# humansensinglab/AGenDA

Hardware: AMD Instinct MI355X
Metric: 512x512 images/sec + DAAM heatmaps, 50 DDIM steps, SD-1.5 (higher is better)
Workload: dtype bf16

## Files before the change

### agenda_amd/_lib.py

```python
from __future__ import annotations

import ctypes as C
import os

_HERE = os.path.dirname(os.path.abspath(__file__))
LIB_PATH = os.environ.get("AGD_LIB") or os.path.join(_HERE, "libagenda_hip.so")
AGD_MAX_LEVELS = 8
AGD_N_CLASSES = 11


class AgdConfig(C.Structure):
    _fields_ = [
        ("struct_size", C.c_int),
        ("in_channels", C.c_int), ("out_channels", C.c_int), ("n_levels", C.c_int),
        ("block_out_channels", C.c_int * AGD_MAX_LEVELS),
        ("down_cross", C.c_int * AGD_MAX_LEVELS),
        ("num_heads", C.c_int * AGD_MAX_LEVELS),
        ("layers_per_block", C.c_int), ("cross_attention_dim", C.c_int),
        ("use_linear_projection", C.c_int), ("norm_num_groups", C.c_int),
        ("vae_latent_channels", C.c_int), ("vae_out_channels", C.c_int), ("vae_n_levels", C.c_int),
        ("vae_block_out_channels", C.c_int * AGD_MAX_LEVELS),
        ("vae_layers_per_block", C.c_int), ("vae_norm_num_groups", C.c_int),
        ("vae_scaling_factor", C.c_float),
        ("max_tokens", C.c_int),
# ... 66 lines not shown
    "agd_inpaint_clear": (C.c_int, [_P]),
    "agd_ip2p_prepare_hw": (C.c_int, [_P, _P, C.c_int, C.c_int, C.c_int, C.c_int, _P, _P]),
    "agd_ip2p_set_hw": (C.c_int, [_P, _P, C.c_int, C.c_int, C.c_int, C.c_float, _P]),
    "agd_ip2p_clear": (C.c_int, [_P]),
    "agd_adapter_configure": (C.c_int, [_P, C.POINTER(AgdAdapterConfig)]),
    "agd_adapter_set_cond_hw": (C.c_int, [_P, _P, C.c_int, C.c_int, C.c_int, C.c_int, _P]),
    "agd_adapter_features": (C.c_int, [_P, _P]),
    "agd_adapter_set_schedule": (C.c_int, [_P, C.POINTER(C.c_float), C.c_int]),
    "agd_adapter_clear": (C.c_int, [_P]),
    "agd_adapter_add_counts": (C.c_int, [_P, C.POINTER(C.c_longlong)]),
    "agd_ip_adapter_begin": (C.c_int, [_P, C.c_int, C.c_int]),
    "agd_ip_adapter_tensor": (C.c_int, [_P, C.c_char_p, _P, C.c_int, C.c_int, C.POINTER(C.c_longlong)]),
    "agd_ip_adapter_commit": (C.c_int, [_P]),
    "agd_ip_adapter_unload": (C.c_int, [_P]),
    "agd_ip_adapter_set": (C.c_int, [_P, _P, C.c_int, C.c_float, _P]),
    "agd_ip_adapter_clear": (C.c_int, [_P]),
    "agd_ip_adapter_tokens": (C.c_int, [_P, _P]),
    "agd_ip_adapter_block": (C.c_int, [_P, C.c_char_p, _P, C.c_int, C.c_int, C.c_int, _P, _P]),
    "agd_ip_adapter_counts": (C.c_int, [_P, C.POINTER(C.c_longlong)]),
    "agd_image_encoder_begin": (C.c_int, [_P, C.POINTER(AgdVisionConfig)]),
    "agd_image_encoder_tensor": (C.c_int, [_P, C.c_char_p, _P, C.c_int, C.c_int, C.POINTER(C.c_longlong)]),
    "agd_image_encoder_commit": (C.c_int, [_P]),
    "agd_image_encoder_unload": (C.c_int, [_P]),
    "agd_image_embeds": (C.c_int, [_P, _P, C.c_int, C.c_int, C.c_int, _P, _P]),
    "agd_gligen_configure": (C.c_int, [_P, C.POINTER(AgdGligenConfig)]),
    "agd_gligen_set": (C.c_int, [_P, _P, _P, _P, C.c_int, _P]),
    "agd_gligen_set_schedule": (C.c_int, [_P, C.POINTER(C.c_int), C.c_int]),
    "agd_gligen_clear": (C.c_int, [_P]),
    "agd_gligen_objs": (C.c_int, [_P, _P]),
    "agd_gligen_fuser": (C.c_int, [_P, C.c_char_p, _P, C.c_int, C.c_int, C.c_int, _P, _P]),
    "agd_lora_add": (C.c_int, [_P, C.c_char_p, _P, _P, C.c_int, C.c_float]),
    "agd_lora_set_scale": (C.c_int, [_P, C.c_float, _P]),
    "agd_lora_clear": (C.c_int, [_P]),
    "agd_lora_count": (C.c_int, [_P]),
    "agd_lora_scale": (C.c_float, [_P]),
    "agd_unet_forward": (C.c_int, [_P, _P, C.c_int, C.c_int, C.c_float, _P, _P]),
    "agd_unet_forward_ts": (C.c_int, [_P, _P, C.c_int, C.c_int, C.POINTER(C.c_float), _P, _P]),
    "agd_cfg_ddim_step": (C.c_int, [_P, _P, _P, C.c_int, C.c_int, C.c_float, C.c_float, C.c_float, _P]),
    "agd_denoise": (C.c_int, [_P, _P, C.c_int, C.c_int, C.c_int, C.POINTER(C.c_float), C.POINTER(C.c_float),
                              C.POINTER(C.c_float), C.c_float, _P]),
    "agd_denoise_plms": (C.c_int, [_P, _P, C.c_int, C.c_int, C.c_int, C.POINTER(C.c_float), C.POINTER(C.c_float),
                                   C.POINTER(C.c_float), C.c_float, _P]),
    "agd_denoise_dpm": (C.c_int, [_P, _P, C.c_int, C.c_int, C.c_int, C.POINTER(C.c_float), C.POINTER(C.c_float), C.c_float, _P]),
    "agd_vae_decode": (C.c_int, [_P, _P, C.c_int, C.c_int, _P, _P, _P]),
    "agd_vae_encode": (C.c_int, [_P, _P, C.c_int, C.c_int, _P, _P, _P]),
    "agd_safety_scores_hw": (C.c_int, [_P, _P, C.c_int, C.c_int, C.c_int, _P, _P, _P]),
    "agd_controlnet_set_cond_hw": (C.c_int, [_P, _P, C.c_int, C.c_int, C.c_int, C.c_int, _P]),
    "agd_controlnet_residuals_hw": (C.c_int, [_P, _P, C.c_int, C.c_int, C.c_int, C.c_float, C.c_float, C.c_int, _P, C.POINTER(C.c_longlong), _P]),
    "agd_inpaint_prepare_hw": (C.c_int, [_P, _P, C.c_int, _P, C.c_int, C.c_int, C.c_int, C.c_int, _P, _P, _P, _P]),
    "agd_inpaint_set_hw": (C.c_int, [_P, _P, C.c_int, _P, C.c_int, _P, C.c_int, C.c_int, C.c_int, _P]),
    "agd_unet_forward_hw": (C.c_int, [_P, _P, C.c_int, C.c_int, C.c_int, C.c_float, _P, _P]),
    "agd_unet_forward_ts_hw": (C.c_int, [_P, _P, C.c_int, C.c_int, C.c_int, C.POINTER(C.c_float), _P, _P]),
    "agd_cfg_ddim_step_hw": (C.c_int, [_P, _P, _P, C.c_int, C.c_int, C.c_int, C.c_float, C.c_float, C.c_float, _P]),
    "agd_denoise_hw": (C.c_int, [_P, _P, C.c_int, C.c_int, C.c_int, C.c_int, C.POINTER(C.c_float), C.POINTER(C.c_float),
                                 C.POINTER(C.c_float), C.c_float, _P]),
    "agd_denoise_plms_hw": (C.c_int, [_P, _P, C.c_int, C.c_int, C.c_int, C.c_int, C.POINTER(C.c_float), C.POINTER(C.c_float),
                                      C.POINTER(C.c_float), C.c_float, _P]),
    "agd_denoise_dpm_hw": (C.c_int, [_P, _P, C.c_int, C.c_int, C.c_int, C.c_int, C.POINTER(C.c_float), C.POINTER(C.c_float), C.c_float, _P]),
    "agd_vae_decode_hw": (C.c_int, [_P, _P, C.c_int, C.c_int, C.c_int, _P, _P, _P]),
    "agd_vae_encode_hw": (C.c_int, [_P, _P, C.c_int, C.c_int, C.c_int, _P, _P, _P]),
    "agd_record_reset_hw": (C.c_int, [_P, C.c_int, C.c_int, C.c_int, _P]),
    "agd_set_option": (C.c_int, [_P, C.c_char_p, C.c_int]),
    "agd_record_config": (C.c_int, [_P, C.c_int, C.c_int, C.c_int]),
    "agd_record_reset": (C.c_int, [_P, C.c_int, C.c_int, _P]),
    "agd_daam_global": (C.c_int, [_P, C.c_int, C.c_int, _P, _P]),
    "agd_hook_global": (C.c_int, [_P, _P, _P]),
    "agd_hook_count": (C.c_int, [_P]),
    "agd_hook_last_map": (C.c_int, [_P, _P, C.c_int, _P]),
    "agd_cross_attn": (C.c_int, [_P, C.c_char_p, _P, _P, C.c_int, C.c_int, C.c_int, _P, C.c_int, _P]),
    "agd_attn_processor": (C.c_int, [_P, C.c_char_p, _P, _P, _P, C.c_int, C.c_int, C.c_int, _P, C.c_int, _P]),
    "agd_hook_reset": (C.c_int, [_P, C.c_int, C.c_int, _P]),
    "agd_hook_num_maps": (C.c_int, [_P]),
    "agd_hook_map_dims": (C.c_int, [_P, C.c_int, C.POINTER(C.c_int)]),
    "agd_hook_map": (C.c_int, [_P, C.c_int, _P, _P]),
    "agd_op_attn_reg_loss": (C.c_int, [_P, C.c_int, C.c_int, C.c_int, _P, _P, _P, C.c_float, _P, _P, _P]),
    "agd_attn_processor_backward": (C.c_int, [_P, C.c_char_p, _P, _P, _P, _P, C.c_int, C.c_int, C.c_int, C.c_int, _P, _P, _P]),
    "agd_op_conv2d": (C.c_int, [_P, _P, _P, _P] + [C.c_int] * 9 + [_P]),
    "agd_op_conv2d_ex": (C.c_int, [_P, _P, _P, _P] + [C.c_int] * 10 + [_P]),
    "agd_op_linear": (C.c_int, [_P, _P, _P, _P, _P, C.c_int, C.c_int, C.c_int, C.c_int, _P]),
    "agd_op_groupnorm": (C.c_int, [_P, _P, _P, _P, C.c_int, C.c_int, C.c_int, C.c_int, C.c_float, C.c_int, _P]),
    "agd_op_conv_groupnorm": (C.c_int, [_P] * 6 + [C.c_int] * 6 + [C.c_float, C.c_int, C.c_int, _P]),
    "agd_op_layernorm": (C.c_int, [_P, _P, _P, _P, C.c_int, C.c_int, C.c_float, _P]),
    "agd_op_ff_fused": (C.c_int, [_P] * 8 + [C.c_int, C.c_int, C.c_float, _P]),
    "agd_op_attn_chain": (C.c_int, [_P] * 9 + [C.c_int] * 5 + [C.c_float, _P]),
    "agd_op_xattn_premul": (C.c_int, [_P] * 9 + [C.c_int] * 5 + [C.c_float, _P]),
    "agd_op_attention": (C.c_int, [_P, _P, _P, _P, C.c_int, C.c_int, C.c_int, C.c_int, C.c_int, C.c_float, _P, _P]),
    "agd_op_attention_headsum": (C.c_int, [_P, _P, _P, _P, C.c_int, C.c_int, C.c_int, C.c_int, C.c_int, C.c_float, _P, _P]),
    "agd_op_bicubic_clamp_mean": (C.c_int, [_P, C.c_int, C.c_int, C.c_int, C.c_int, _P, _P]),
    "agd_op_heatmap_u8": (C.c_int, [_P, C.c_int, C.c_int, _P, _P]),
    "agd_op_resize_u8_pil": (C.c_int, [_P, C.c_int, C.c_int, C.c_int, C.c_int, C.c_int, C.c_int, _P, _P]),
    "agd_op_stack_heatmaps": (C.c_int, [_P, _P, _P, C.c_longlong, _P, _P, _P]),
    "agd_op_window_gather": (C.c_int, [_P, _P] + [C.c_int] * 8 + [_P]),
    "agd_op_window_mean": (C.c_int, [_P, _P] + [C.c_int] * 6 + [_P]),
    "agd_denoise_panorama": (C.c_int, [_P, _P] + [C.c_int] * 7 + [C.POINTER(C.c_float)] * 3 + [C.c_float, _P]),
    "agd_daam_global_panorama": (C.c_int, [_P, C.c_int, C.c_int, _P, _P]),
    "agd_freeu_set": (C.c_int, [_P] + [C.c_float] * 4),
    "agd_freeu_clear": (C.c_int, [_P]),
    "agd_freeu_counts": (C.c_int, [_P, C.POINTER(C.c_longlong)]),
    "agd_op_freeu": (C.c_int, [_P, _P, _P, _P] + [C.c_int] * 5 + [C.c_float, C.c_float, _P]),
    "agd_profile_begin": (C.c_int, [_P]),
    "agd_profile_end": (C.c_int, [_P, C.POINTER(C.c_double), C.POINTER(C.c_double), C.POINTER(C.c_longlong)]),
    "agd_profile_end_ex": (C.c_int, [_P, C.c_double, C.c_double] + [C.POINTER(C.c_double)] * 5 + [C.POINTER(C.c_longlong)]),
    "agd_profile_class_name": (C.c_char_p, [C.c_int]),
    "agd_version": (C.c_char_p, []),
}

EXPORTS = tuple(_SIGS.keys())
_lib = None


def load():
    global _lib
    if _lib is not None:
        return _lib
    if not os.path.exists(LIB_PATH):
        raise AgendaHipError(
            f"{LIB_PATH} not found: build it with `python -c 'import __graft_entry__ as g; g.build()'` "
            "or `make -C agenda_amd/csrc`. There is no CPU fallback.")
    lib = C.CDLL(LIB_PATH)
    for name, (res, args) in _SIGS.items():
        fn = getattr(lib, name)
        fn.restype = res
        fn.argtypes = args
    _lib = lib
    return lib


def check(rc: int, ctx=None, what: str = ""):
    if rc != 0:
        msg = load().agd_last_error(ctx)
        raise AgendaHipError(f"{what} failed (rc={rc}): {msg.decode() if msg else '?'}")


def ptr(t):
    if t is None:
        return None
    assert t.is_contiguous(), "tensor must be contiguous"
    return C.c_void_p(t.data_ptr())


def current_stream_ptr():
    import torch
    return C.c_void_p(torch.cuda.current_stream().cuda_stream)
```

### agenda_amd/csrc/kernels.h

```cpp
#pragma once
#include "common.h"

#define AGD_MAX_DEVICES 16
struct SplitKWs { float* p = nullptr; size_t cap = 0; };

struct IgemmP {
  const bf16_t* sc0 = nullptr; const bf16_t* sc1 = nullptr; int sc_C0 = 0, sc_C1 = 0;
  int ups4 = 0;
  const bf16_t* src0; const bf16_t* src1;
  int C0, C1;
  int Hin, Win, Hout, Wout;
  int ksize, stride, pad, up;
  const bf16_t* W;
  const float* bias; int bias_mode;
  const float* rowadd; int rowadd_ld;
  const bf16_t* residual; int ldr;
  void* out; int out_f32; int ldo;
  int M, N, K;
  float alpha;
  int geglu;
  int act;
  int batch;
  long long sA0, sA1, sW, sO, sR;
  const bf16_t* zero_page;
  SplitKWs* ws;
  float* splitk_ws;
  int colstat_rows;
  float* colstat_out;
  float* rowstat_out; int rowstat_slots;
  const float* ln_stats; int ln_slots; const float* ln_cs; float ln_invC, ln_eps;
  int* cfg_out;
  int w_per_image;
  int wmajor;
  int warm;
  int halo;
  int p8;
  const float* gn_gamma; const float* gn_beta; bf16_t* gn_y; int gn_groups; float gn_eps; int gn_silu; int gn_keep_out; int* gn_fused;
  int kg2;
  int smap;
  int wreg, wreg_mmin, wreg_mmax;
  const bf16_t* Wfrag; int wfrag_ni;
  int xb_m, xb_n;
  int xcd_block;
  int pc;
  int stagger;
  int dbg;
};
int launch_igemm(const IgemmP& p, hipStream_t st);
int igemm_query(const IgemmP& p, int* cfg3);

struct AttnP {
  const bf16_t* q; const bf16_t* k; const bf16_t* v; bf16_t* o;
  int ldq, ldk, ldv, ldo;
  long long sq, sk, sv, so;
  int B, H, D, Nq, Nk;
  float scale;
  int record_mode; int rec_b0;
  float* rec; long long rec_img_stride; long long rec_head_stride;
  int rec_T;
  int rec_hpb;
  int nqt;
  int causal;
  const float* mask;
  const bf16_t* k2; const bf16_t* v2; int ldk2, ldv2; long long sk2, sv2; int Nk2;
};
int launch_attention(const AttnP& p, hipStream_t st);

struct FFusedP {
  const bf16_t* h; bf16_t* out;
  const bf16_t* w1f;
  const float* cs1; const float* b1;
  const bf16_t* w2f;
  const float* b2;
  int M; float ln_eps;
  const bf16_t* wpf; const float* bp; const bf16_t* xres; bf16_t* pout; float* colstat;
  int xres_rows;
  int premul;
};
int launch_ff_fused(const FFusedP& p, int C, hipStream_t st);
struct AttnChainP {
  const bf16_t* h; bf16_t* out;
  const float* gamma; const float* beta; float ln_eps;
  const bf16_t* wqf;
  const bf16_t* wof; const float* bo;
  const bf16_t* kv; int ldkv; long long skv;
  int M, HW, T; float scale;
  int record; float* rec; long long rec_img_stride, rec_head_stride; int rec_T, rec_b0, rec_hpb;
  float* rowstat_out;
  const bf16_t* o1; const bf16_t* wo1f; const float* bo1;
  int rows32;
  int src_rows;
};
int launch_attn_chain(const AttnChainP& p, int C, int heads, hipStream_t st);
struct QkvChainP {
  const bf16_t* x;
  const bf16_t* wbf; long long wb_stride; const float* rowadd;
  bf16_t* h;
  const float* gamma; const float* beta; float ln_eps;
  const bf16_t* wqkvf;
  bf16_t* qkv;
  int M, HW;
  long long rowadd_stride;
  const float* gn_part; int gn_bm, gn_groups; float gn_eps; const float* gn_gamma; const float* gn_beta;
  int rows64;
  int sched2;
};
int launch_qkv_chain(const QkvChainP& p, int C, hipStream_t st);
int launch_frag_order_w1(const bf16_t* src, bf16_t* dst, int C, int HID, hipStream_t st);
int launch_frag_order_w(const bf16_t* src, bf16_t* dst, int N, int K, int NI, int KC, hipStream_t st);

#define XATTN_TP 80
struct XattnPremulP {
  const bf16_t* kv; int ldkv; long long skv;
  const bf16_t* wqT;
  const bf16_t* wo;
  const float* gamma; const float* wqb;
  int B, T, C, H; float scale;
  bf16_t* kpp; float* kcs; float* kbs; bf16_t* vpp;
};
int launch_xattn_premul(const XattnPremulP& p, hipStream_t st);
struct XattnSP {
  const bf16_t* x;
  const float* ln_stats; int ln_slots; float ln_invC, ln_eps;
  const bf16_t* kpp; const float* kcs; const float* kbs;
  bf16_t* P;
  int M, HW, C, H, T;
  float* rec; long long rec_img_stride, rec_head_stride; int rec_T, rec_b0;
};
int launch_xattn_s(const XattnSP& p, hipStream_t st);
int launch_matvec_bf16(const bf16_t* W, const float* v, float* out, int N, int K, hipStream_t st);
int launch_rowstat_bf16(const bf16_t* x, float* out, int M, int C, hipStream_t st);

struct GroupNormP {
  const bf16_t* x0; const bf16_t* x1; int C0, C1;
  bf16_t* y;
  const float* gamma; const float* beta;
  int B, HW, groups; float eps; int silu;
  float* ws;
  const float* part0; const float* part1; int bm0, bm1;
};
int launch_groupnorm(const GroupNormP& p, hipStream_t st);
int launch_gn_fold_weight(const float* part, int bm, int B, int HW, int C, int groups, float eps, const float* gamma, const float* beta,
                          const bf16_t* W, const float* bias, int N, bf16_t* Wb, float* rowadd, hipStream_t st, int frag_ni = 0);
long long groupnorm_ws_floats(int B, int C, int HW, int groups);
int launch_layernorm(const bf16_t* x, bf16_t* y, const float* g, const float* b, int rows, int C, float eps, hipStream_t st);

int launch_convert_weight(const float* w, bf16_t* out, int N, int Cin, int taps, int Cpad, int geglu_bn, hipStream_t st);
int launch_f32_to_bf16(const float* x, bf16_t* y, long long n, hipStream_t st);
int launch_bf16_to_f32(const bf16_t* x, float* y, long long n, hipStream_t st);
bool igemm_can_fuse_shortcut(const IgemmP& p);
int launch_upsample_phase_weight(const bf16_t* w, bf16_t* out, int Cout, int Cin, hipStream_t st);
int launch_prep_latents(const float* lat_nchw, bf16_t* out_nhwc, int B, int C, int HW, int Cpad, int dup, float scale, hipStream_t st);
int launch_timestep_embed(float t, float* out, int dim, hipStream_t st);
int launch_small_linear(const float* x, const bf16_t* W, const float* bias, float* out, int M, int N, int K, int silu_in,
                        int silu_out, hipStream_t st);
int launch_cfg_ddim(const float* eps_nhwc, int ldc, float* lat_nchw, int B, int C, int HW, float guidance,
                    float a_t, float a_p, int vpred, hipStream_t st);
int launch_cfg_plms(const float* eps_nhwc, int ldc, float* lat, const float* src, const float* h1, const float* h2, const float* h3,
                    float* store, int B, int C, int HW, float guidance, const float* w4, float a, float b, hipStream_t st);
int launch_cfg_dpm(const float* eps_nhwc, int ldc, float* lat, const float* prev, float* store, int B, int C, int HW, float guidance,
// ... 89 lines not shown
```

### agenda_amd/csrc/model.hip

```cpp
#include "../../include/agenda_hip.h"
#include "kernels.h"

#include <algorithm>
#include <cmath>
#include <cstdarg>
#include <cstdio>
#include <cstring>
#include <functional>
#include <string>
#include <unordered_map>
#include <vector>

static thread_local char g_err[2048] = "";
#define AGD_API extern "C" __attribute__((visibility("default")))
extern "C" void agd_set_error(const char* fmt, ...) {
  va_list ap; va_start(ap, fmt); vsnprintf(g_err, sizeof(g_err), fmt, ap); va_end(ap);
}
#define CK(expr) do { if ((expr) != 0) return -1; } while (0)
#define FAIL(...) do { agd_set_error(__VA_ARGS__); return -1; } while (0)

struct WMat { bf16_t* w = nullptr; int N = 0, Cin = 0, Cpad = 0, taps = 0;
              int sc_cols = 0;
              bf16_t* wfrag = nullptr; int wfrag_ni = 0; };
struct Act { bf16_t* p = nullptr; int B = 0, H = 0, W = 0, C = 0; float* cpart = nullptr; int cpart_bm = 0;
             bf16_t* normed = nullptr; const float* normed_gamma = nullptr;
             long long n() const { return (long long)B * H * W * C; } };
struct NextGn { const float* gamma = nullptr; const float* beta = nullptr; float eps = 0.f; int silu = 0; };

struct Arena {
  char* base = nullptr; size_t cap = 0, off = 0, peak = 0;
  void* alloc(size_t bytes) {
    size_t a = (off + 255) & ~(size_t)255;
    if (a + bytes > cap) { agd_set_error("activation arena exhausted: need %zu + %zu > %zu bytes (raise workspace_bytes)", a, bytes, cap); return nullptr; }
    off = a + bytes; if (off > peak) peak = off;
    return base + a;
  }
  size_t mark() const { return off; }
  void release(size_t m) { off = m; }
};

enum { PC_CONV3 = 0, PC_GEMM, PC_ATTN_SELF, PC_ATTN_CROSS, PC_GN, PC_LN, PC_ELEM, PC_HEAT, PC_VAE_ATTN, PC_OTHER, PC_TOUCH };
static const char* kClassNames[AGD_N_CLASSES] = {"igemm_conv3x3", "igemm_linear_1x1", "attn_self_flash", "attn_cross_daam",
                                                 "groupnorm", "layernorm", "elementwise", "heatmap", "vae_attn_softmax", "other", "weight_touch"};

struct DBuf {
  void* p = nullptr; size_t cap = 0;
  template <typename T> T* as() const { return (T*)p; }
  int ensure(size_t bytes) {
    if (p && bytes <= cap) return 0;
    if (p) { (void)hipDeviceSynchronize(); (void)hipFree(p); p = nullptr; cap = 0; }
    const size_t want = bytes ? bytes : 256;
    if (hipMalloc(&p, want) != hipSuccess) { p = nullptr; agd_set_error("hipMalloc(%zu) failed", want); return -1; }
    cap = want;
    return 0;
  }
  void release() { if (p) (void)hipFree(p); p = nullptr; cap = 0; }
};

struct XLayer {
  std::string name; int C = 0, heads = 0, level = 0; bool mid = false;
  bool cn = false;
  WMat wkv; DBuf kvb; bf16_t* kv = nullptr; DBuf accb; float* acc = nullptr; int acc_h = 0, acc_w = 0;
  int acc_heads = 0;
  DBuf wqTb, wkvTb, woTb; WMat wqT, wkvT, woT;
  bf16_t* pm_wqT = nullptr; float* pm_wqb = nullptr; bool pm_ready = false;
  DBuf pm_kppb, pm_vppb, pm_csb; bf16_t* pm_kpp = nullptr; bf16_t* pm_vpp = nullptr; float* pm_kcs = nullptr; float* pm_kbs = nullptr;
};

struct Fuser {
  std::string pre; int C = 0, heads = 0;
  WMat wqkv, wkv; float ta = 0.f, td = 0.f; float* bo_s = nullptr; float* b2_s = nullptr;
  DBuf gkvb;
};

struct IpaLayer {
  std::string pre; int C = 0, heads = 0, cols = 0;
  DBuf wk, wv, kppb, vppb, csbsb;
};

enum : int {
  TBF_FF            = 1 << 0,
  TBF_ATTN2         = 1 << 1,
  TBF_ATTN1_OUT     = 1 << 2,
  TBF_FF_PROJ       = 1 << 3,
  TBF_QKV           = 1 << 4,
  TBF_ATTN2_640     = 1 << 5,
  TBF_LAZY_DUP      = 1 << 6,
  TBF_QKV_GN        = 1 << 7,
  TBF_QKV_640       = 1 << 8,
  TBF_FF_PREMUL     = 1 << 9,
  TBF_ATTN2_ROWS32  = 1 << 10,
  TBF_QKV_ROWS64    = 1 << 11,
  TBF_QKV_SCHED2    = 1 << 12,
  TBF_DEFAULT       = 0x1fff & ~TBF_QKV_640,
};

struct ProfEv { int cls; double flops, bytes; hipEvent_t a, b; };

struct EvalCond {
  float cn_scale = 0.f;
  bool grounded = false;
  float ad_scale = 0.f;
  bool ipa = false;
};

struct agd_ctx {
  int device = 0; agd_config cfg{}; std::string err;
  std::unordered_map<std::string, WMat> W;
  std::unordered_map<std::string, float*> V;
  std::unordered_map<std::string, int> Vn;
  std::vector<void*> owned;
  Arena arena; bf16_t* zero_page = nullptr;
  float* stage = nullptr; size_t stage_bytes = 0;
  bool finalized = false;
  WMat tproj_all; float* tproj_bias = nullptr; float* tproj_out = nullptr; int tproj_total = 0;
  const float* tproj_cur = nullptr;
  int tproj_cur_ld = 0;
  float* tsteps_buf = nullptr; int tsteps_cap = 0;
  std::unordered_map<std::string, int> tproj_off;
  float* temb_buf = nullptr;
  float* t_dev = nullptr;
  std::vector<XLayer> xl; std::unordered_map<std::string, int> xl_idx;
  DBuf ctxb; bf16_t* ctx_bf16 = nullptr; int ctx_B2 = 0, ctx_T = 0;
  int rec_mode = 0, rec_is_train = 0, rec_T_cfg = 0, rec_T = 0, rec_B = 0, rec_L = 0, rec_Lh = 0, rec_Lw = 0;
  DBuf hook_sumb, hook_scratchb, hook_headsb, hook_storeb;
  struct HookRec { size_t off; int Bp, T, N; };
  std::vector<HookRec> hook_recs; size_t hook_store_used = 0;
  DBuf bwd_wsb;
  float* hook_sum = nullptr; float* hook_scratch = nullptr; int hook_count = 0, hook_Bp = 0, hook_T = 0;
  int rec_base = 0, rec_call = 0;
  int pano_B = 0, pano_Lh = 0, pano_Lw = 0, pano_stride = 0;
  DBuf pano_ctxb;
  DBuf pano_viewb, pano_hmb;
  DBuf latb, epsb, vae_imgb, plmsb, dpmb;
  bf16_t* lat_bf16 = nullptr; float* eps_nhwc = nullptr;
  SplitKWs splitk;
  int opt_cfg_share = 1;
  int opt_ln_fold = 1;
  int opt_gn_fused = 1;
  int opt_warm = 3;
  int opt_gn_proj_fold = 1;
  int opt_p8 = 1;
  int opt_halo = 1;
  int opt_tb_fuse = TBF_DEFAULT;
  int opt_ups4 = 7;
  int opt_ffproj = 1;
  int opt_sc_fuse = 3;
  int opt_wreg = 3;
  int opt_kg2 = 1;
  int opt_side = 0;
  hipStream_t side = nullptr; hipEvent_t ev_fork = nullptr, ev_join = nullptr;
  int opt_smap = 1;
  int opt_reduce_gn = 1;
  int opt_xcd_block = 1;
  int opt_pc = 49;
  agd_vision_config vis{}; bool vis_on = false; float* vis_concepts = nullptr;
  agd_vision_config ienc{}; int ienc_state = 0;
  int opt_xpre = 1;
  int opt_touch = 3;
  unsigned* touch_sink = nullptr;
  agd_controlnet_config cnc{}; bool cn_on = false;
  WMat cn_tproj_all; float* cn_tproj_bias = nullptr; float* cn_tproj_out = nullptr; int cn_tproj_total = 0;
  int cn_nres = 0; float* cn_zb = nullptr; float* cn_zbs = nullptr; int cn_zb_total = 0; std::vector<int> cn_zb_off; float cn_zscale = NAN;
  DBuf cn_embb; int cn_emb_B2 = 0, cn_emb_Lh = 0, cn_emb_Lw = 0, cn_emb_rep = 0;
  std::vector<float> cn_sched;
  int ip_mode = 0, ip_B = 0, ip_Lh = 0, ip_Lw = 0, ip_Cm = 0, ip_Cc = 0;
  DBuf ip_maskb, ip_condb, ip_noiseb;
  std::vector<float> ip_sched;
  bool i2_on = false; int i2_B = 0, i2_Lh = 0, i2_Lw = 0; float i2_scale = 1.f;
  int i2_prep_B = 0, i2_prep_Lh = 0, i2_prep_Lw = 0;
  DBuf i2_latb;
  std::vector<std::string> lora_keys; std::vector<LoraMergeD> lora_d; int lora_tiles = 0;
  DBuf lora_descb; bf16_t* lora_scratch = nullptr; size_t lora_scratch_n = 0;
  float lora_scale = 0.f; bool lora_dirty = false;
  bool ctx_stale = false;
  agd_gligen_config glc{}; bool gl_on = false;
  std::vector<Fuser> gl_f; std::unordered_map<std::string, int> gl_idx;
// ... 317 lines not shown
      a.rec_head_stride = (long long)T * N; a.rec_img_stride = a.rec_head_stride * xl.heads;
      hook_call = true;
    }
  }
  CK(run_attention(c, st, PC_ATTN_CROSS, a));
  if (hook_call) {
    ProfScope ps(c, st, PC_HEAT, 0);
    CK(launch_hook_headmean(c->hook_headsb.as<float>(), c->hook_Bp, xl.heads, T, N, c->hook_scratch, st));
    if (c->rec_is_train) {
      const size_t bytes = (size_t)c->hook_Bp * T * N * 4, need = c->hook_store_used + bytes;
      if (need > c->hook_storeb.cap) {
        DBuf bigger; CK(bigger.ensure(need * 2 > ((size_t)64 << 20) ? need * 2 : ((size_t)64 << 20)));
        if (c->hook_store_used && hipMemcpyAsync(bigger.p, c->hook_storeb.p, c->hook_store_used, hipMemcpyDeviceToDevice, st) != hipSuccess) FAIL("hook store copy");
        hipStreamSynchronize(st);
        c->hook_storeb.release(); c->hook_storeb = bigger;
      }
      if (hipMemcpyAsync((char*)c->hook_storeb.p + c->hook_store_used, c->hook_scratch, bytes, hipMemcpyDeviceToDevice, st) != hipSuccess) FAIL("hook store");
      c->hook_recs.push_back({c->hook_store_used, c->hook_Bp, T, N});
      c->hook_store_used = need;
    }
    CK(launch_hook_accum(c->hook_scratch, c->hook_Bp, T, side, c->rec_L, c->hook_sum, st));
    c->hook_count++;
  }
  return 0;
}

static int fuser_rows(agd_ctx* c, hipStream_t st, const Fuser& f, bf16_t* h, int B, int HW, bf16_t* qkv, bf16_t* att,
                      const std::function<int(const bf16_t*, int, const WMat&, const GemmOpt&)>& last) {
  const int C = f.C, D = C / f.heads, M = B * HW, NO = c->glc.max_objs;
  if (B != c->gl_B2) FAIL("gligen: the grounding objects are set for %d rows, this forward has %d (agd_gligen_set)", c->gl_B2, B);
  const std::string t = f.pre + "transformer_blocks.0.fuser.";
  bf16_t* n = (bf16_t*)c->arena.alloc((size_t)M * C * 2); bf16_t* ff = (bf16_t*)c->arena.alloc((size_t)M * 4 * C * 2);
  if (!n || !ff) return -1;
  GETV(g1, t + "norm1.weight"); GETV(b1, t + "norm1.bias"); GETV(g2, t + "norm2.weight"); GETV(b2, t + "norm2.bias");
  GETW(wo, t + "attn.to_out.0.weight"); GETW(w1, t + "ff.net.0.proj.weight"); GETV(bb1, t + "ff.net.0.proj.bias"); GETW(w2, t + "ff.net.2.weight");
  { ProfScope ps(c, st, PC_LN, 0, 4.0 * M * (double)C); CK(launch_layernorm(h, n, g1, b1, M, C, 1e-5f, st)); }
  { GemmOpt o; CK(run_conv(c, st, n, C, nullptr, 0, 1, 1, M, f.wqkv, 1, qkv, o, c->zero_page)); }
  AttnP a{}; a.q = qkv; a.k = qkv + C; a.v = qkv + 2 * C; a.o = att;
  a.ldq = a.ldk = a.ldv = 3 * C; a.ldo = C; a.sq = a.sk = a.sv = (long long)HW * 3 * C; a.so = (long long)HW * C;
  a.B = B; a.H = f.heads; a.D = D; a.Nq = HW; a.Nk = HW; a.scale = 1.0f / sqrtf((float)D);
  a.k2 = f.gkvb.as<bf16_t>(); a.v2 = a.k2 + C; a.ldk2 = a.ldv2 = 2 * C; a.sk2 = a.sv2 = (long long)NO * 2 * C; a.Nk2 = NO;
  { const double fl = 4.0 * B * f.heads * (double)HW * (HW + NO) * D, by = 2.0 * B * (double)C * (4.0 * HW + 2.0 * NO);
    ProfScope ps(c, st, PC_ATTN_SELF, fl, by); CK(launch_attention(a, st)); }
  { GemmOpt o; o.bias = f.bo_s; o.alpha = f.ta; o.residual = h; CK(run_conv(c, st, att, C, nullptr, 0, 1, 1, M, *wo, 1, h, o, c->zero_page)); }
  { ProfScope ps(c, st, PC_LN, 0, 4.0 * M * (double)C); CK(launch_layernorm(h, n, g2, b2, M, C, 1e-5f, st)); }
  { GemmOpt o; o.bias = bb1; o.geglu = 1; CK(run_conv(c, st, n, C, nullptr, 0, 1, 1, M, *w1, 1, ff, o, c->zero_page)); }
  GemmOpt o; o.bias = f.b2_s; o.alpha = f.td; o.residual = h;
  return last(ff, 4 * C, *w2, o);
}

static int dup_half(agd_ctx* c, hipStream_t st, bf16_t* p, long long half_elems) {
  ProfScope ps(c, st, PC_ELEM, 0);
  if (hipMemcpyAsync(p + half_elems, p, (size_t)half_elems * 2, hipMemcpyDeviceToDevice, st) != hipSuccess) FAIL("dup_half copy failed");
  return 0;
}

enum TbHead  { HEAD_GN,
               HEAD_FOLD,
               HEAD_QKV,
               HEAD_QKV_GN };
enum TbDup   { DUP_NONE, DUP_COPY,
               DUP_LAZY };
enum TbAttn2 { ATTN2_CHAIN,
               ATTN2_PREMUL,
               ATTN2_KERNELS };
enum TbFf    { FF_FUSED,
               FF_FUSED_PROJ,
               FF_FUSED_PREMUL,
               FF_FFPROJ,
               FF_PLAIN };

struct TBlockPlan {
  bool fold;
  bool x_normed;
  bool gfold;
  TbHead head; int qkv_rows64, qkv_sched2;
  bool attn1_in_chain;
  TbDup dup;
  const Fuser* fuser;
  const IpaLayer* ipa;
  XLayer* xl;
  TbAttn2 attn2; int chain_rows32;
  bool daam;
  TbFf ff;
  bool wreg_proj;
  bool stats_head, stats_attn1, stats_attn2;
  bool stats_ipa;
};

static const float kTbLnEps = 1e-5f;

struct TBlock {
  agd_ctx* c; hipStream_t st; const std::string& pre; const std::string t; const Act& x; Act& out; int heads, groups;
  int C, HW, Bs, B;
  const float* gn_g = nullptr; const float* gn_b = nullptr; const WMat* w_in = nullptr; const float* b_in = nullptr;
  bf16_t* ln = nullptr;
  bf16_t* h = nullptr; bf16_t* qkv = nullptr; bf16_t* att = nullptr;
  const bf16_t* xres;
  int M; const int Mshared;
  float* stats = nullptr; int slots = 0;
  bf16_t* ipaP = nullptr;
  TBlock(agd_ctx* c_, hipStream_t st_, const std::string& pre_, const Act& x_, Act& out_, int heads_, int groups_, int dup)
    : c(c_), st(st_), pre(pre_), t(pre_ + "transformer_blocks.0."), x(x_), out(out_), heads(heads_), groups(groups_), C(x_.C), HW(x_.H * x_.W),
      Bs(x_.B), B(dup ? 2 * x_.B : x_.B), xres(x_.p), M(x_.B * x_.H * x_.W), Mshared(M) {}

  int produce(const bf16_t* A, int K, const WMat& w, GemmOpt o, bool shaped, bool want_stats) {
    const int gb_ = shaped ? M / HW : 1, gh_ = shaped ? x.H : 1, gw_ = shaped ? x.W : M;
    stats = nullptr; slots = 0;
    if (want_stats) {
      int cfg[3] = {0, 0, 0}; GemmOpt qo = o; qo.query_cfg = cfg; qo.want_rowstat = 1;
      CK(run_conv(c, st, A, K, nullptr, 0, gb_, gh_, gw_, w, 1, h, qo, c->zero_page));
      slots = (w.N + cfg[1] - 1) / cfg[1];
      stats = (float*)c->arena.alloc((size_t)B * HW * slots * 2 * sizeof(float)); if (!stats) return -1;
      o.rowstat_out = stats; o.rowstat_slots = slots;
    }
    return run_conv(c, st, A, K, nullptr, 0, gb_, gh_, gw_, w, 1, h, o, c->zero_page);
  }
  int consume(bool fold, const std::string& lnkey, const std::string& wkey, const float* bias, int geglu, bf16_t* outp) {
    if (fold) {
      const std::string k = wkey + ".lnfold";
      GETW(wf, k); GETV(cs, k + ".cs"); GETV(bf, k + ".bias");
      GemmOpt o; o.bias = bf; o.geglu = geglu; o.ln_stats = stats; o.ln_slots = slots; o.ln_cs = cs; o.ln_invC = 1.0f / (float)C; o.ln_eps = kTbLnEps;
      if (geglu && C == 1280 && M >= 1024 && M <= 4096 && (c->opt_wreg & 1) && wf->wfrag) o.wreg = 2;
      return run_conv(c, st, h, C, nullptr, 0, 1, 1, M, *wf, 1, outp, o, c->zero_page);
    }
    GETV(g, lnkey + ".weight"); GETV(b, lnkey + ".bias");
    { ProfScope ps(c, st, PC_LN, 0, 4.0 * M * (double)C); CK(launch_layernorm(h, ln, g, b, M, C, kTbLnEps, st)); }
    GETW(w, wkey); GemmOpt o; o.bias = bias; o.geglu = geglu;
    return run_conv(c, st, ln, C, nullptr, 0, 1, 1, M, *w, 1, outp, o, c->zero_page);
  }
};

static TBlockPlan tblock_plan(const TBlock& s, int dup) {
  agd_ctx* c = s.c; const Act& x = s.x; const std::string& pre = s.pre; const std::string& t = s.t;
  const int C = s.C, HW = s.HW, heads = s.heads, groups = s.groups;
  auto tb = [c](int bit) { return (c->opt_tb_fuse & bit) != 0; };
  auto has = [c](const std::string& key) { return c->W.count(key) != 0; };
  TBlockPlan p{};
  p.fold = c->opt_ln_fold == 1 || (c->opt_ln_fold == 2 && C <= 320) || (c->opt_ln_fold == 3 && C <= 640);
  p.x_normed = x.normed && x.normed_gamma == s.gn_g;
  p.wreg_proj = C == 640 && (c->opt_wreg & 2);
  const bool sums = c->opt_gn_fused && x.cpart && x.cpart_bm > 0 && HW % x.cpart_bm == 0;
  p.gfold = c->opt_gn_proj_fold && sums && C <= (c->opt_gn_proj_fold >= 2 ? 640 : 320) && HW % 128 == 0;
  if (p.gfold) {
    const bool qkv = tb(TBF_QKV) && C == 320 && s.w_in->N == C && has(t + "attn1.qkv.frag");
    const bool gn_inside = qkv && tb(TBF_QKV_GN) && groups <= 32 && has(pre + "proj_in.frag");
    p.head = gn_inside ? HEAD_QKV_GN : qkv ? HEAD_QKV : HEAD_FOLD;
    p.qkv_rows64 = qkv && tb(TBF_QKV_ROWS64) && HW % 64 == 0;
  } else if (C == 640 && tb(TBF_QKV) && tb(TBF_QKV_640) && tb(TBF_QKV_GN) && sums && HW % 64 == 0 && groups <= 32 && !p.x_normed && !dup &&
             has(pre + "proj_in.frag") && has(t + "attn1.qkv.frag")) {
    p.head = HEAD_QKV_GN;
  } else p.head = HEAD_GN;
  p.qkv_sched2 = tb(TBF_QKV_SCHED2);
  const bool ff_fused = tb(TBF_FF) && p.fold && C == 320 && has(t + "ff.w1.frag");
  if (ff_fused) {
    const bool proj = tb(TBF_FF_PROJ) && has(pre + "proj_out.frag");
    p.ff = !proj ? FF_FUSED : tb(TBF_FF_PREMUL) && has(t + "ff.w2p.frag") ? FF_FUSED_PREMUL : FF_FUSED_PROJ;
  } else p.ff = c->opt_ffproj && has(pre + "ffproj.weight") ? FF_FFPROJ : FF_PLAIN;
  auto itx = c->xl_idx.find(t + "attn2");
  p.xl = itx == c->xl_idx.end() ? nullptr : &c->xl[itx->second];
  p.daam = p.xl && daam_records(c, *p.xl, s.B, x.H, x.W);
  const bool premul = p.xl && p.xl->pm_ready && c->opt_xpre && p.fold && HW % 64 == 0 && c->rec_mode != 2 && c->ctx_T <= XATTN_TP && !dup &&
                      (!p.daam || p.xl->acc_heads == p.xl->heads);
  const bool chain = !premul && tb(TBF_ATTN2) && (C == 320 || (C == 640 && tb(TBF_ATTN2_640))) && heads == 8 && HW % (C == 320 ? 128 : 64) == 0 &&
                     c->ctx_T <= 96 && c->rec_mode != 2 && has(t + "attn2.to_q.frag");
  p.attn2 = premul ? ATTN2_PREMUL : chain ? ATTN2_CHAIN : ATTN2_KERNELS;
  p.chain_rows32 = tb(TBF_ATTN2_ROWS32);
  if (c->cur.grounded) { auto itf = c->gl_idx.find(pre); if (itf != c->gl_idx.end()) p.fuser = &c->gl_f[itf->second]; }
  if (c->cur.ipa) { auto iti = c->ipa_idx.find(pre); if (iti != c->ipa_idx.end()) p.ipa = &c->ipa_l[iti->second]; }
  const bool lazy = dup && tb(TBF_LAZY_DUP) && chain && C == 320 && (p.ff == FF_FUSED_PROJ || p.ff == FF_FUSED_PREMUL) && !p.fuser && !p.ipa;
  p.dup = !dup ? DUP_NONE : lazy ? DUP_LAZY : DUP_COPY;
  p.attn1_in_chain = chain && tb(TBF_ATTN1_OUT) && p.dup != DUP_COPY && has(t + "attn1.to_out.frag") && !p.fuser && !p.ipa;
  p.stats_head = p.fold; p.stats_attn1 = p.fold && !chain; p.stats_attn2 = p.fold && !ff_fused && !p.ipa; p.stats_ipa = p.fold && !ff_fused && p.ipa;
  return p;
}

static int qkv_chain_params(const TBlock& s, const TBlockPlan& p, const bf16_t* wb, const float* radd, QkvChainP& qp) {
  agd_ctx* c = s.c; const Act& x = s.x; const int C = s.C;
  GETW(fqkv, s.t + "attn1.qkv.frag"); GETV(g1, s.t + "norm1.weight"); GETV(b1, s.t + "norm1.bias");
  qp.x = x.p; qp.wbf = wb; qp.wb_stride = (long long)s.w_in->N * C; qp.rowadd = radd; qp.rowadd_stride = C; qp.h = s.h; qp.gamma = g1; qp.beta = b1; qp.ln_eps = kTbLnEps;
  qp.wqkvf = fqkv->w; qp.qkv = s.qkv; qp.M = s.M; qp.HW = s.HW; qp.rows64 = p.qkv_rows64; qp.sched2 = p.qkv_sched2;
  if (p.head == HEAD_QKV_GN) {
    GETW(fpi, s.pre + "proj_in.frag");
    if (!s.b_in) FAIL("proj_in without bias");
    qp.wbf = fpi->w; qp.wb_stride = 0; qp.rowadd = s.b_in; qp.rowadd_stride = 0;
    qp.gn_part = x.cpart; qp.gn_bm = x.cpart_bm; qp.gn_groups = s.groups; qp.gn_eps = 1e-6f; qp.gn_gamma = s.gn_g; qp.gn_beta = s.gn_b;
  }
  return 0;
}

static int tb_head(TBlock& s, const TBlockPlan& p) {
  agd_ctx* c = s.c; hipStream_t st = s.st; const Act& x = s.x; const WMat* w = s.w_in; const int C = s.C;
  if (p.head == HEAD_GN) {
    if (p.x_normed) s.ln = x.normed;
    else CK(run_gn(c, st, x.p, C, nullptr, 0, s.Bs, s.HW, s.gn_g, s.gn_b, s.groups, 1e-6f, 0, s.ln, &x));
    GemmOpt o; o.bias = s.b_in;
    if (p.wreg_proj) o.wreg = 1;
    return s.produce(s.ln, C, *w, o, false, p.stats_head);
  }
  if (p.gfold) { if (w->taps != 1 || w->Cpad != C) FAIL("gn_proj_fold: proj_in weight [N=%d taps=%d Cpad=%d] is not a 1x1 over %d channels", w->N, w->taps, w->Cpad, C); }
  else if (w->taps != 1 || w->Cpad != C || w->N != C || !s.b_in) FAIL("qkv chain: proj_in weight [N=%d taps=%d Cpad=%d] is not a biased 1x1 over %d channels", w->N, w->taps, w->Cpad, C);
  bf16_t* wb = nullptr; float* radd = nullptr;
  if (p.head != HEAD_QKV_GN) {
    wb = (bf16_t*)c->arena.alloc((size_t)s.Bs * w->N * C * 2);
    radd = (float*)c->arena.alloc((size_t)s.Bs * w->N * sizeof(float));
    if (!wb || !radd) return -1;
    ProfScope ps(c, st, PC_GN, 0, 2.0 * s.Bs * (double)w->N * C * 2);
    CK(launch_gn_fold_weight(x.cpart, x.cpart_bm, s.Bs, s.HW, C, s.groups, 1e-6f, s.gn_g, s.gn_b, w->w, s.b_in, w->N, wb, radd, st, p.head == HEAD_QKV ? C / 64 : 0));
  }
  if (p.head == HEAD_FOLD) {
    WMat wi = *w; wi.w = wb;
    GemmOpt o; o.rowadd = radd; o.rowadd_ld = w->N; o.w_per_image = 1;
    return s.produce(x.p, C, wi, o, true, p.stats_head);
  }
  QkvChainP qp{}; CK(qkv_chain_params(s, p, wb, radd, qp));
  s.stats = nullptr; s.slots = 0;
  ProfScope ps(c, st, PC_GEMM, 8.0 * s.M * (double)C * C, 2.0 * s.M * (double)C * 5.0 + 2.0 * (p.gfold ? s.Bs + 3.0 : 4.0) * C * (double)C);
  return launch_qkv_chain(qp, C, st);
}

static int tb_self_attention(TBlock& s, const TBlockPlan& p) {
  agd_ctx* c = s.c; const std::string& t = s.t; const int C = s.C, HW = s.HW, D = C / s.heads;
  if (p.head == HEAD_GN || p.head == HEAD_FOLD) CK(s.consume(p.fold, t + "norm1", t + "attn1.qkv", nullptr, 0, s.qkv));
  AttnP a{}; a.q = s.qkv; a.k = s.qkv + C; a.v = s.qkv + 2 * C; a.o = s.att;
  a.ldq = a.ldk = a.ldv = 3 * C; a.ldo = C; a.sq = a.sk = a.sv = (long long)HW * 3 * C; a.so = (long long)HW * C;
  a.B = s.Bs; a.H = s.heads; a.D = D; a.Nq = HW; a.Nk = HW; a.scale = 1.0f / sqrtf((float)D);
  CK(run_attention(c, s.st, PC_ATTN_SELF, a));
  if (p.attn1_in_chain) return 0;
  GETW(wo, t + "attn1.to_out.0.weight"); GETV(bo, t + "attn1.to_out.0.bias");
  GemmOpt oo; oo.bias = bo; oo.residual = s.h;
  return s.produce(s.att, C, *wo, oo, false, p.stats_attn1);
}

static int tb_duplicate(TBlock& s, const TBlockPlan& p) {
  agd_ctx* c = s.c; hipStream_t st = s.st; const int C = s.C, M = s.Mshared;
  if (p.dup == DUP_NONE) return 0;
  s.M = s.B * s.HW;
  if (p.dup == DUP_LAZY) return 0;
  CK(dup_half(c, st, s.h, (long long)M * C));
  if (p.stats_attn1) { ProfScope ps(c, st, PC_ELEM, 0);
// ... 45 lines not shown
  return 0;
}

static int tb_attn2_chain(TBlock& s, const TBlockPlan& p) {
  agd_ctx* c = s.c; const std::string& t = s.t; const XLayer& xl = *p.xl; const int C = s.C, HW = s.HW, B = s.B, M = s.M, heads = s.heads;
  GETW(fq, t + "attn2.to_q.frag"); GETW(fo, t + "attn2.to_out.frag");
  GETV(g2, t + "norm2.weight"); GETV(b2, t + "norm2.bias"); GETV(bo, t + "attn2.to_out.0.bias");
  const int T = c->ctx_T, D = C / heads;
  AttnChainP ap{}; ap.h = s.h; ap.out = s.h; ap.gamma = g2; ap.beta = b2; ap.ln_eps = kTbLnEps; ap.wqf = fq->w; ap.wof = fo->w; ap.bo = bo;
  ap.kv = xl.kv; ap.ldkv = 2 * C; ap.skv = (long long)T * 2 * C; ap.M = M; ap.HW = HW; ap.T = T; ap.scale = 1.0f / sqrtf((float)D);
  double rec_bytes = 0;
  if (p.daam) {
    ap.record = 1; ap.rec_b0 = B / 2; ap.rec_T = c->rec_T; ap.rec_hpb = heads / xl.acc_heads;
    ap.rec_head_stride = (long long)c->rec_T * HW; ap.rec_img_stride = ap.rec_head_stride * xl.acc_heads;
    ap.rec = xl.acc + (size_t)c->rec_base * ap.rec_img_stride;
    rec_bytes = 8.0 * (B - ap.rec_b0) * xl.acc_heads * (double)c->rec_T * HW;
  }
  if (p.attn1_in_chain || p.dup == DUP_LAZY) {
    ap.out = (bf16_t*)c->arena.alloc((size_t)M * C * 2); if (!ap.out) return -1;
  }
  if (p.attn1_in_chain) {
    GETW(f1o, t + "attn1.to_out.frag"); GETV(bo1, t + "attn1.to_out.0.bias");
    ap.o1 = s.att; ap.wo1f = f1o->w; ap.bo1 = bo1;
  }
  if (p.dup == DUP_LAZY) ap.src_rows = s.Mshared;
  ap.rows32 = p.chain_rows32;
  if (p.stats_attn2) {
    s.slots = 1; s.stats = (float*)c->arena.alloc((size_t)M * 2 * sizeof(float)); if (!s.stats) return -1;
    ap.rowstat_out = s.stats;
  }
  const double gemms = p.attn1_in_chain ? 6.0 : 4.0;
  ProfScope ps(c, s.st, PC_ATTN_CROSS, gemms * M * (double)C * C + 4.0 * B * heads * (double)HW * T * D, gemms * M * (double)C + gemms * C * (double)C + 4.0 * B * (double)T * C + rec_bytes);
  CK(launch_attn_chain(ap, C, heads, s.st));
  s.h = ap.out;
  return 0;
}

static int tb_attn2_premul(TBlock& s, const TBlockPlan& p) {
  agd_ctx* c = s.c; const XLayer& xl = *p.xl; const int C = s.C, HW = s.HW, B = s.B, M = s.M, heads = s.heads;
  if (!s.stats || s.slots <= 0) FAIL("attn2_premul: the GEMM in front of attn2 left no row statistics for norm2");
  GETV(bo, s.t + "attn2.to_out.0.bias");
  const int HT = heads * XATTN_TP;
  bf16_t* P = (bf16_t*)c->arena.alloc((size_t)M * HT * 2); if (!P) return -1;
  XattnSP sp{}; sp.x = s.h; sp.ln_stats = s.stats; sp.ln_slots = s.slots; sp.ln_invC = 1.0f / (float)C; sp.ln_eps = kTbLnEps;
  sp.kpp = xl.pm_kpp; sp.kcs = xl.pm_kcs; sp.kbs = xl.pm_kbs; sp.P = P; sp.M = M; sp.HW = HW; sp.C = C; sp.H = heads; sp.T = c->ctx_T;
  double rec_bytes = 0;
  if (p.daam) {
    sp.rec_b0 = B / 2; sp.rec_T = c->rec_T; sp.rec_head_stride = (long long)c->rec_T * HW; sp.rec_img_stride = sp.rec_head_stride * xl.acc_heads;
    sp.rec = xl.acc + (size_t)c->rec_base * sp.rec_img_stride;
    rec_bytes = 8.0 * (B - sp.rec_b0) * heads * (double)c->rec_T * HW;
  }
  { ProfScope ps(c, s.st, PC_ATTN_CROSS, 2.0 * M * (double)HT * C, 2.0 * M * (double)C + 2.0 * B * (double)HT * C + 2.0 * M * (double)HT + rec_bytes);
    CK(launch_xattn_s(sp, s.st)); }
  WMat wv; wv.w = xl.pm_vpp; wv.N = C; wv.Cin = HT; wv.Cpad = HT; wv.taps = 1;
  GemmOpt oo; oo.bias = bo; oo.residual = s.h; oo.w_per_image = 1;
  return s.produce(P, HT, wv, oo, true, p.stats_attn2);
}

static int tb_attn2(TBlock& s, const TBlockPlan& p) {
  agd_ctx* c = s.c; const std::string& t = s.t;
  if (!p.xl) FAIL("cross-attn layer %s not registered", (t + "attn2").c_str());
  if (c->ctx_B2 != s.B) FAIL("context batch %d != unet batch %d (call agd_set_context)", c->ctx_B2, s.B);
  if (p.attn2 == ATTN2_CHAIN) return tb_attn2_chain(s, p);
  if (p.attn2 == ATTN2_PREMUL) return tb_attn2_premul(s, p);
  CK(s.consume(p.fold, t + "norm2", t + "attn2.to_q.weight", nullptr, 0, s.qkv));
  CK(cross_attention(c, s.st, *p.xl, s.qkv, s.B, s.HW, s.x.H, s.x.W, s.att, true));
  GETW(wo, t + "attn2.to_out.0.weight"); GETV(bo, t + "attn2.to_out.0.bias");
  GemmOpt oo; oo.bias = bo; oo.residual = s.h;
  return s.produce(s.att, s.C, *wo, oo, false, p.stats_attn2);
}

static int tb_ff_fused(TBlock& s, const TBlockPlan& p) {
  agd_ctx* c = s.c; const std::string& t = s.t; Act& out = s.out; const int C = s.C, M = s.M;
  GETW(f1, t + "ff.w1.frag"); GETW(f2, t + "ff.w2.frag");
  const std::string k = t + "ff.net.0.proj.weight.lnfold";
  GETV(cs, k + ".cs"); GETV(bf, k + ".bias"); GETV(b2, t + "ff.net.2.bias");
  FFusedP fp{}; fp.h = s.h; fp.out = s.h; fp.w1f = f1->w; fp.cs1 = cs; fp.b1 = bf; fp.w2f = f2->w; fp.b2 = b2; fp.M = M; fp.ln_eps = kTbLnEps;
  const bool proj = p.ff != FF_FUSED;
  if (proj) {
    GETW(fpw, s.pre + "proj_out.frag"); GETV(bp, s.pre + "proj_out.bias");
    fp.wpf = fpw->w; fp.bp = bp; fp.xres = s.xres; fp.pout = out.p;
    if (p.ff == FF_FUSED_PREMUL) {
      GETW(f2p, t + "ff.w2p.frag"); GETV(bcp, s.pre + "ffproj.bias");
      fp.w2f = f2p->w; fp.bp = bcp; fp.premul = 1;
    }
    if (p.dup == DUP_LAZY) fp.xres_rows = s.Mshared;
    out.cpart_bm = 0;
    if (out.cpart && c->opt_gn_fused && s.HW % 128 == 0) { fp.colstat = out.cpart; out.cpart_bm = 128; }
  }
  ProfScope ps(c, s.st, PC_GEMM, 2.0 * M * (double)C * (proj ? 13.0 : 12.0) * C, (proj ? 8.0 : 4.0) * M * (double)C + 2.0 * (proj ? 13.0 : 12.0) * C * (double)C);
  return launch_ff_fused(fp, C, s.st);
}

static int tb_feed_forward(TBlock& s, const TBlockPlan& p) {
  agd_ctx* c = s.c; hipStream_t st = s.st; const std::string& t = s.t; const int C = s.C, M = s.M;
  if (p.ff == FF_FUSED || p.ff == FF_FUSED_PROJ || p.ff == FF_FUSED_PREMUL) CK(tb_ff_fused(s, p));
  else {
    bf16_t* ff = (bf16_t*)c->arena.alloc((size_t)M * 4 * C * 2); if (!ff) return -1;
    GETV(b1, t + "ff.net.0.proj.bias");
    CK(s.consume(p.fold, t + "norm3", t + "ff.net.0.proj.weight", b1, 1, ff));
    if (p.ff == FF_FFPROJ) {
      GETW(wc, s.pre + "ffproj.weight"); GETV(bc, s.pre + "ffproj.bias");
      GemmOpt o; o.bias = bc; o.residual = s.xres; o.out_act = &s.out; o.rows_per_image = s.HW;
      return run_conv(c, st, ff, 4 * C, s.h, C, 1, 1, M, *wc, 1, s.out.p, o, c->zero_page);
    }
    GETW(w2, t + "ff.net.2.weight"); GETV(b2, t + "ff.net.2.bias");
    GemmOpt o2; o2.bias = b2; o2.residual = s.h;
    CK(run_conv(c, st, ff, 4 * C, nullptr, 0, 1, 1, M, *w2, 1, s.h, o2, c->zero_page));
  }
  if (p.ff != FF_FUSED && p.ff != FF_PLAIN) return 0;
  GETW(w, s.pre + "proj_out.weight"); GETV(b, s.pre + "proj_out.bias");
  GemmOpt o; o.bias = b; o.residual = s.xres; o.out_act = &s.out; o.rows_per_image = s.HW;
  if (p.wreg_proj) o.wreg = 1;
  return run_conv(c, st, s.h, C, nullptr, 0, 1, 1, M, *w, 1, s.out.p, o, c->zero_page);
}

static int transformer(agd_ctx* c, hipStream_t st, const std::string& pre, const Act& x, int heads, int groups, Act& out, int dup = 0) {
  TBlock s(c, st, pre, x, out, heads, groups, dup);
  const int B = s.B, HW = s.HW, C = s.C;
  out = alloc_act(c, B, x.H, x.W, C, true); if (!out.p) return -1;
  const size_t mk = c->arena.mark();
  Act n = alloc_act(c, B, x.H, x.W, C); if (!n.p) return -1;
  Act h = alloc_act(c, B, x.H, x.W, C); if (!h.p) return -1;
  s.ln = n.p; s.h = h.p;
  s.qkv = (bf16_t*)c->arena.alloc((size_t)B * HW * 3 * C * 2); if (!s.qkv) return -1;
  s.att = (bf16_t*)c->arena.alloc((size_t)B * HW * C * 2); if (!s.att) return -1;
  GETV(gg, pre + "norm.weight"); GETV(gb, pre + "norm.bias"); GETW(w_in, pre + "proj_in.weight"); GETV(b_in, pre + "proj_in.bias");
  s.gn_g = gg; s.gn_b = gb; s.w_in = w_in; s.b_in = b_in;
  const TBlockPlan p = tblock_plan(s, dup);
  CK(tb_head(s, p));
  CK(tb_self_attention(s, p));
  CK(tb_duplicate(s, p));
  if (p.fuser) CK(tb_fuser(s, p));
  if (p.ipa) CK(tb_ip_adapter_scores(s, p));
  CK(tb_attn2(s, p));
  if (p.ipa) CK(tb_ip_adapter_add(s, p));
  CK(tb_feed_forward(s, p));
  c->arena.release(mk);
  return 0;
}

static int time_embed(agd_ctx* c, hipStream_t st, const float* ts, int n, float* scratch, float* out, bool cn = false) {
  const int dim = c->cfg.block_out_channels[0], td = dim * 4;
  const std::string pre = cn ? "controlnet." : "unet.";
  ProfScope ps(c, st, PC_ELEM, 0);
  float* e0 = scratch; float* e1 = e0 + (size_t)n * dim; float* e2 = e1 + (size_t)n * td;
  for (int i = 0; i < n; ++i) CK(launch_timestep_embed(ts[i], e0 + (size_t)i * dim, dim, st));
  GETW(w1, pre + "time_embedding.linear_1.weight"); GETV(b1, pre + "time_embedding.linear_1.bias");
  GETW(w2, pre + "time_embedding.linear_2.weight"); GETV(b2, pre + "time_embedding.linear_2.bias");
  CK(launch_small_linear(e0, w1->w, b1, e1, n, td, w1->Cpad, 0, 1, st));
  CK(launch_small_linear(e1, w2->w, b2, e2, n, td, w2->Cpad, 0, 0, st));
  if (cn) CK(launch_small_linear(e2, c->cn_tproj_all.w, c->cn_tproj_bias, out, n, c->cn_tproj_total, td, 1, 0, st));
  else CK(launch_small_linear(e2, c->tproj_all.w, c->tproj_bias, out, n, c->tproj_total, td, 1, 0, st));
  return 0;
}

static int adapter_add(agd_ctx* c, hipStream_t st, int level, const Act& h, Act& out);
static int down_mid_walk(agd_ctx* c, hipStream_t st, const std::string& u, const bf16_t* xin, int B2, int Lh, int Lw, bool shared,
                         const bf16_t* conv_in_res, const std::function<int(const Act&)>& on_sample, Act& h) {
  const agd_config& g = c->cfg;
  const int nl = g.n_levels, G = g.norm_num_groups;
  const int Bh = shared ? B2 / 2 : B2;
  const bool inject = c->cur.ad_scale != 0.f && u == "unet.";
  h = alloc_act(c, B2, Lh, Lw, g.block_out_channels[0], true); if (!h.p) return -1;
  { GETW(w, u + "conv_in.weight"); GETV(b, u + "conv_in.bias"); GemmOpt o; o.bias = b; o.out_act = &h; o.residual = conv_in_res;
    CK(run_conv(c, st, xin, 64, nullptr, 0, Bh, Lh, Lw, *w, 3, h.p, o, c->zero_page)); }
  if (shared) {
// ... 1753 lines not shown
AGD_API int agd_op_groupnorm(const float* x, const float* gamma, const float* beta, float* y, int B, int C, int HW, int groups,
                                float eps, int silu, void* stream) {
  hipStream_t st = S(stream); Tmp tmp;
  bf16_t* xb = tmp.get<bf16_t>((size_t)B * HW * C); bf16_t* yb = tmp.get<bf16_t>((size_t)B * HW * C);
  float* ws = tmp.get<float>((size_t)groupnorm_ws_floats(B, C, HW, groups)); float* yf = tmp.get<float>((size_t)B * HW * C);
  if (!xb || !yb || !ws || !yf) return -1;
  CK(to_nhwc_bf16(x, xb, B, C, HW, C, st));
  GroupNormP g{}; g.x0 = xb; g.C0 = C; g.y = yb; g.gamma = gamma; g.beta = beta; g.B = B; g.HW = HW; g.groups = groups; g.eps = eps; g.silu = silu; g.ws = ws;
  CK(launch_groupnorm(g, st));
  CK(launch_bf16_to_f32(yb, yf, (long long)B * HW * C, st));
  CK(launch_nchw_from_nhwc_f32(yf, C, y, B, C, HW, st));
  hipStreamSynchronize(st);
  return 0;
}

AGD_API int agd_op_conv_groupnorm(const float* x, const float* w, const float* bias, const float* gamma, const float* beta, float* y, int B,
                                  int Cin, int H, int W, int Cout, int groups, float eps, int silu, int fused, void* stream) {
  hipStream_t st = S(stream); Tmp tmp;
  const int Cpad = (Cin + 63) / 64 * 64, HW = H * W;
  bf16_t* xb = tmp.get<bf16_t>((size_t)B * HW * Cpad); bf16_t* wb = tmp.get<bf16_t>((size_t)Cout * 9 * Cpad);
  bf16_t* hb = tmp.get<bf16_t>((size_t)B * HW * Cout); bf16_t* yb = tmp.get<bf16_t>((size_t)B * HW * Cout);
  float* part = tmp.get<float>((size_t)((long long)B * HW / 64 + 1) * Cout * 2); float* yf = tmp.get<float>((size_t)B * HW * Cout);
  float* ws = tmp.get<float>((size_t)groupnorm_ws_floats(B, Cout, HW, groups));
  if (!xb || !wb || !hb || !yb || !part || !yf || !ws) return -1;
  CK(to_nhwc_bf16(x, xb, B, Cin, HW, Cpad, st));
  CK(launch_convert_weight(w, wb, Cout, Cin, 9, Cpad, 0, st));
  IgemmP p{};
  p.src0 = xb; p.C0 = Cpad; p.Hin = H; p.Win = W; p.Hout = H; p.Wout = W; p.ksize = 3; p.stride = 1; p.pad = 1; p.up = 1;
  p.W = wb; p.bias = bias; p.bias_mode = bias ? 1 : 0; p.N = Cout; p.K = 9 * Cpad; p.M = B * HW; p.ldr = Cout; p.out = hb; p.ldo = Cout;
  p.alpha = 1.f; p.batch = 1; p.zero_page = op_zero_page();
  p.p8 = (fused & 4) ? 2 : (fused & 8) ? 3 : (fused & 2) ? 1 : 0; fused &= 1;
  int bm = 0;
  if (fused) {
    int cfg[3] = {0, 0, 0};
    CK(igemm_query(p, cfg));
    bm = cfg[0];
    if (cfg[2] != 1 || bm < 1 || HW % bm || HW % 64) { agd_set_error("op_conv_groupnorm: shape not eligible for producer statistics (tile %d, splits %d)", cfg[0], cfg[2]); return -1; }
    p.colstat_out = part; p.colstat_rows = HW;
  }
  CK(launch_igemm(p, st));
  GroupNormP g{}; g.x0 = hb; g.C0 = Cout; g.y = yb; g.gamma = gamma; g.beta = beta; g.B = B; g.HW = HW; g.groups = groups; g.eps = eps; g.silu = silu; g.ws = ws;
  if (fused) { g.part0 = part; g.bm0 = bm; }
  CK(launch_groupnorm(g, st));
  CK(launch_bf16_to_f32(yb, yf, (long long)B * HW * Cout, st));
  CK(launch_nchw_from_nhwc_f32(yf, Cout, y, B, Cout, HW, st));
  hipStreamSynchronize(st);
  return 0;
}

AGD_API int agd_op_layernorm(const float* x, const float* gamma, const float* beta, float* y, int rows, int C, float eps, void* stream) {
  hipStream_t st = S(stream); Tmp tmp;
  bf16_t* xb = tmp.get<bf16_t>((size_t)rows * C); bf16_t* yb = tmp.get<bf16_t>((size_t)rows * C);
  if (!xb || !yb) return -1;
  CK(launch_f32_to_bf16(x, xb, (long long)rows * C, st));
  CK(launch_layernorm(xb, yb, gamma, beta, rows, C, eps, st));
  CK(launch_bf16_to_f32(yb, y, (long long)rows * C, st));
  hipStreamSynchronize(st);
  return 0;
}

AGD_API int agd_op_ff_fused(const float* x, const float* gamma, const float* beta, const float* w1, const float* b1, const float* w2,
                            const float* b2, float* y, int M, int C, float eps, void* stream) {
  hipStream_t st = S(stream); Tmp tmp;
  if (C != 320) { agd_set_error("op_ff_fused: C = %d (320 only)", C); return -1; }
  const int H8 = 8 * C, H4 = 4 * C;
  bf16_t* xb = tmp.get<bf16_t>((size_t)M * C); bf16_t* yb = tmp.get<bf16_t>((size_t)M * C);
  bf16_t* w1b = tmp.get<bf16_t>((size_t)H8 * C); bf16_t* w1l = tmp.get<bf16_t>((size_t)H8 * C); bf16_t* w1f = tmp.get<bf16_t>((size_t)H8 * C);
  bf16_t* w2b = tmp.get<bf16_t>((size_t)C * H4); bf16_t* w2f = tmp.get<bf16_t>((size_t)C * H4);
  float* cs = tmp.get<float>(H8); float* bf = tmp.get<float>(H8);
  if (!xb || !yb || !w1b || !w1l || !w1f || !w2b || !w2f || !cs || !bf) return -1;
  CK(launch_f32_to_bf16(x, xb, (long long)M * C, st));
  CK(launch_convert_weight(w1, w1b, H8, C, 1, C, 16, st));
  CK(launch_ln_fold_weight(w1b, gamma, beta, b1, H8, C, 16, w1l, cs, bf, st));
  CK(launch_frag_order_w1(w1l, w1f, C, H4, st));
  CK(launch_convert_weight(w2, w2b, C, H4, 1, H4, 0, st));
  CK(launch_frag_order_w(w2b, w2f, C, H4, C / 64, 128, st));
  FFusedP fp{}; fp.h = xb; fp.out = yb; fp.w1f = w1f; fp.cs1 = cs; fp.b1 = bf; fp.w2f = w2f; fp.b2 = b2; fp.M = M; fp.ln_eps = eps;
  CK(launch_ff_fused(fp, C, st));
  CK(launch_bf16_to_f32(yb, y, (long long)M * C, st));
  hipStreamSynchronize(st);
  return 0;
}

AGD_API int agd_op_attn_chain(const float* x, const float* gamma, const float* beta, const float* wq, const float* kv, const float* wo,
                              const float* bo, float* y, float* probs_sum, int B, int HW, int T, int C, int heads, float eps, void* stream) {
  hipStream_t st = S(stream); Tmp tmp;
  const long long M = (long long)B * HW;
  bf16_t* xb = tmp.get<bf16_t>((size_t)M * C); bf16_t* yb = tmp.get<bf16_t>((size_t)M * C); bf16_t* kvb = tmp.get<bf16_t>((size_t)B * T * 2 * C);
  bf16_t* wqb = tmp.get<bf16_t>((size_t)C * C); bf16_t* wqf = tmp.get<bf16_t>((size_t)C * C);
  bf16_t* wob = tmp.get<bf16_t>((size_t)C * C); bf16_t* wof = tmp.get<bf16_t>((size_t)C * C);
  if (!xb || !yb || !kvb || !wqb || !wqf || !wob || !wof) return -1;
  if (C != 320 && C != 640) { agd_set_error("op_attn_chain: C %d", C); return -1; }
  CK(launch_f32_to_bf16(x, xb, M * C, st));
  CK(launch_f32_to_bf16(kv, kvb, (long long)B * T * 2 * C, st));
  CK(launch_convert_weight(wq, wqb, C, C, 1, C, 0, st)); CK(launch_frag_order_w(wqb, wqf, C, C, 5, C, st));
  CK(launch_convert_weight(wo, wob, C, C, 1, C, 0, st)); CK(launch_frag_order_w(wob, wof, C, C, 5, C, st));
  AttnChainP ap{}; ap.h = xb; ap.out = yb; ap.gamma = gamma; ap.beta = beta; ap.ln_eps = eps; ap.wqf = wqf; ap.wof = wof; ap.bo = bo;
  ap.rows32 = (heads >> 8) & 1; heads &= 255;
  ap.kv = kvb; ap.ldkv = 2 * C; ap.skv = (long long)T * 2 * C; ap.M = (int)M; ap.HW = HW; ap.T = T; ap.scale = 1.0f / sqrtf((float)(C / heads));
  if (probs_sum) {
    if (hipMemsetAsync(probs_sum, 0, (size_t)B * T * HW * 4, st) != hipSuccess) { agd_set_error("memset probs"); return -1; }
    ap.record = 1; ap.rec = probs_sum; ap.rec_b0 = 0; ap.rec_T = T; ap.rec_hpb = heads; ap.rec_head_stride = (long long)T * HW; ap.rec_img_stride = (long long)T * HW;
  }
  CK(launch_attn_chain(ap, C, heads, st));
  CK(launch_bf16_to_f32(yb, y, M * C, st));
  hipStreamSynchronize(st);
  return 0;
}

AGD_API int agd_op_xattn_premul(const float* x, const float* gamma, const float* beta, const float* wq, const float* kv, const float* wo,
                                const float* bo, float* y, float* probs, int B, int HW, int T, int C, int heads, float eps, void* stream) {
  hipStream_t st = S(stream); Tmp tmp;
  const long long M = (long long)B * HW;
  if (heads < 1 || C % heads || (C / heads) % 8 || C % 160 || C % 64 || HW % 64 || T < 1 || T > XATTN_TP || (heads * XATTN_TP) % 64) { agd_set_error("op_xattn_premul: C %d heads %d HW %d T %d", C, heads, HW, T); return -1; }
  const size_t HT = (size_t)heads * XATTN_TP;
  bf16_t* xb = tmp.get<bf16_t>((size_t)M * C); bf16_t* yb = tmp.get<bf16_t>((size_t)M * C); bf16_t* kvb = tmp.get<bf16_t>((size_t)B * T * 2 * C);
  bf16_t* wqb = tmp.get<bf16_t>((size_t)C * C); bf16_t* wqT = tmp.get<bf16_t>((size_t)C * C); bf16_t* wob = tmp.get<bf16_t>((size_t)C * C);
  float* wqbeta = tmp.get<float>(C); float* rst = tmp.get<float>((size_t)M * 2);
  bf16_t* kpp = tmp.get<bf16_t>((size_t)B * HT * C); bf16_t* vpp = tmp.get<bf16_t>((size_t)B * HT * C); float* kcs = tmp.get<float>((size_t)B * HT * 2);
  bf16_t* P = tmp.get<bf16_t>((size_t)M * HT);
  if (!xb || !yb || !kvb || !wqb || !wqT || !wob || !wqbeta || !rst || !kpp || !vpp || !kcs || !P) return -1;
  CK(launch_f32_to_bf16(x, xb, M * C, st));
  CK(launch_f32_to_bf16(kv, kvb, (long long)B * T * 2 * C, st));
  CK(launch_convert_weight(wq, wqb, C, C, 1, C, 0, st)); CK(launch_transpose_bf16(wqb, C, C, wqT, st));
  CK(launch_convert_weight(wo, wob, C, C, 1, C, 0, st));
  CK(launch_matvec_bf16(wqb, beta, wqbeta, C, C, st));
  CK(launch_rowstat_bf16(xb, rst, (int)M, C, st));
  XattnPremulP pm{}; pm.kv = kvb; pm.ldkv = 2 * C; pm.skv = (long long)T * 2 * C; pm.wqT = wqT; pm.wo = wob; pm.gamma = gamma; pm.wqb = wqbeta;
  pm.B = B; pm.T = T; pm.C = C; pm.H = heads; pm.scale = 1.0f / sqrtf((float)(C / heads)); pm.kpp = kpp; pm.kcs = kcs; pm.kbs = kcs + (size_t)B * HT; pm.vpp = vpp;
  CK(launch_xattn_premul(pm, st));
  XattnSP sp{}; sp.x = xb; sp.ln_stats = rst; sp.ln_slots = 1; sp.ln_invC = 1.0f / (float)C; sp.ln_eps = eps; sp.kpp = kpp; sp.kcs = pm.kcs; sp.kbs = pm.kbs; sp.P = P;
  sp.M = (int)M; sp.HW = HW; sp.C = C; sp.H = heads; sp.T = T;
  if (probs) {
    if (hipMemsetAsync(probs, 0, (size_t)B * heads * T * HW * 4, st) != hipSuccess) { agd_set_error("memset probs"); return -1; }
    sp.rec = probs; sp.rec_b0 = 0; sp.rec_T = T; sp.rec_head_stride = (long long)T * HW; sp.rec_img_stride = sp.rec_head_stride * heads;
  }
  CK(launch_xattn_s(sp, st));
  WMat wv; wv.w = vpp; wv.N = C; wv.Cin = (int)HT; wv.Cpad = (int)HT; wv.taps = 1;
  GemmOpt oo; oo.bias = bo; oo.residual = xb; oo.w_per_image = 1;
  CK(run_conv(nullptr, st, P, (int)HT, nullptr, 0, B, 1, HW, wv, 1, yb, oo, op_zero_page()));
  CK(launch_bf16_to_f32(yb, y, M * C, st));
  hipStreamSynchronize(st);
  return 0;
}

AGD_API int agd_op_attention(const float* q, const float* k, const float* v, float* o, int B, int H, int D, int Nq, int Nk,
                                float scale, float* probs_out, void* stream) {
  hipStream_t st = S(stream); Tmp tmp;
  const int C = H * D;
  bf16_t* qb = tmp.get<bf16_t>((size_t)B * Nq * C); bf16_t* kb = tmp.get<bf16_t>((size_t)B * Nk * C);
  bf16_t* vb = tmp.get<bf16_t>((size_t)B * Nk * C); bf16_t* ob = tmp.get<bf16_t>((size_t)B * Nq * C);
  if (!qb || !kb || !vb || !ob) return -1;
  CK(launch_f32_to_bf16(q, qb, (long long)B * Nq * C, st));
  CK(launch_f32_to_bf16(k, kb, (long long)B * Nk * C, st));
  CK(launch_f32_to_bf16(v, vb, (long long)B * Nk * C, st));
  AttnP a{}; a.q = qb; a.k = kb; a.v = vb; a.o = ob; a.ldq = a.ldk = a.ldv = a.ldo = C;
  a.sq = (long long)Nq * C; a.so = a.sq; a.sk = (long long)Nk * C; a.sv = a.sk;
  a.B = B; a.H = H; a.D = D; a.Nq = Nq; a.Nk = Nk; a.scale = scale;
  if (probs_out) {
    if (hipMemsetAsync(probs_out, 0, (size_t)B * H * Nk * Nq * 4, st) != hipSuccess) { agd_set_error("memset probs"); return -1; }
    a.record_mode = 1; a.rec_b0 = 0; a.rec = probs_out; a.rec_T = Nk;
    a.rec_head_stride = (long long)Nk * Nq; a.rec_img_stride = a.rec_head_stride * H;
  }
  CK(launch_attention(a, st));
  CK(launch_bf16_to_f32(ob, o, (long long)B * Nq * C, st));
  hipStreamSynchronize(st);
// ... 70 lines not shown
  fill_rand(w, (long long)Cout * taps * Ctot, 3, 0.05f); if (r) fill_rand(r, M * Nout, 4, 1.0f);
  hipMemset(bias, 0, Cout * 4);
  WMat wm; wm.w = w; wm.N = Cout; wm.Cin = Ctot; wm.Cpad = Ctot; wm.taps = taps;
  const int mode = geglu; geglu &= 1;
  GemmOpt o; o.bias = bias; o.stride = stride; o.up = up; o.geglu = geglu; o.residual = r; o.halo = (mode & 8) ? 1 : 0;
  o.p8 = (mode & 32) ? 2 : (mode & 64) ? 3 : (mode & 16) ? 1 : 0;
  o.smap = (mode & 256) ? 1 : 0;
  o.kg2 = (mode & 512) ? 1 : 0;
  o.pc = ((mode >> 11) & 15) | ((mode >> 12) & 48);
  o.xcd_block = (mode >> 15) & 1;
  if (mode & 128) {
    const int ni = geglu ? 4 : 2;
    wm.wfrag = tmp.get<bf16_t>((size_t)Cout * taps * Ctot); if (!wm.wfrag) return -1;
    if (taps != 1 || C1) { agd_set_error("bench: wreg is for plain 1x1 launches"); return -1; }
    CK(launch_frag_order_w(w, wm.wfrag, Cout, Ctot, ni, Ctot, 0));
    wm.wfrag_ni = ni; o.wreg = (mode & 1024) ? 7 : 3;
  }
  float* stats = nullptr; float* cs = nullptr;
  if (mode & 6) {
    int cfg[3] = {0, 0, 0}; GemmOpt qo = o; qo.query_cfg = cfg; qo.want_rowstat = (mode & 2) ? 1 : 0;
    CK(run_conv(nullptr, 0, x0, C0, x1, C1, B, H, W, wm, ksize, y, qo, op_zero_page()));
    const int slots = (mode & 2) ? (Cout + cfg[1] - 1) / cfg[1] : 2;
    stats = tmp.get<float>((size_t)M * slots * 2); cs = tmp.get<float>(Cout);
    if (!stats || !cs) return -1;
    hipMemset(stats, 0, (size_t)M * slots * 2 * 4); hipMemset(cs, 0, Cout * 4);
    if (mode & 2) { o.rowstat_out = stats; o.rowstat_slots = slots; }
    if (mode & 4) { o.ln_stats = stats; o.ln_slots = slots; o.ln_cs = cs; o.ln_invC = 1.0f / Ctot; o.ln_eps = 1e-5f; }
  }
  hipEvent_t a, b; hipEventCreate(&a); hipEventCreate(&b);
  for (int i = 0; i < 2; ++i) CK(run_conv(nullptr, 0, x0, C0, x1, C1, B, H, W, wm, ksize, y, o, op_zero_page()));
  hipEventRecord(a, 0);
  for (int i = 0; i < iters; ++i) CK(run_conv(nullptr, 0, x0, C0, x1, C1, B, H, W, wm, ksize, y, o, op_zero_page()));
  hipEventRecord(b, 0); hipEventSynchronize(b);
  float t = 0; hipEventElapsedTime(&t, a, b);
  *ms_out = t / iters;
  hipEventDestroy(a); hipEventDestroy(b);
  return 0;
}

AGD_API int agd_bench_conv_cold(int B, int H, int W, int C0, int Cout, int ksize, int geglu, int with_residual, int warm, int iters, double* ms_out) {
  Tmp tmp;
  const int taps = ksize * ksize;
  const long long M = (long long)B * H * W;
  const int Nout = geglu ? Cout / 2 : Cout;
  const size_t xn = (size_t)M * C0, wn = (size_t)Cout * taps * C0, flush_bytes = (size_t)1 << 30;
  bf16_t* x0 = tmp.get<bf16_t>(xn); bf16_t* xs = tmp.get<bf16_t>(xn); bf16_t* w = tmp.get<bf16_t>(wn); bf16_t* y = tmp.get<bf16_t>((size_t)M * Nout);
  bf16_t* r = with_residual ? tmp.get<bf16_t>((size_t)M * Nout) : nullptr;
  float* bias = tmp.get<float>(Cout); char* scratch = tmp.get<char>(flush_bytes); unsigned* sink = tmp.get<unsigned>(64);
  if (!x0 || !xs || !w || !y || !bias || !scratch || !sink || (with_residual && !r)) return -1;
  fill_rand(xs, (long long)xn, 1, 1.0f); fill_rand(w, (long long)wn, 3, 0.05f); if (r) fill_rand(r, M * Nout, 4, 1.0f);
  hipMemset(bias, 0, Cout * 4);
  WMat wm; wm.w = w; wm.N = Cout; wm.Cin = C0; wm.Cpad = C0; wm.taps = taps;
  GemmOpt o; o.bias = bias; o.geglu = geglu; o.residual = r; o.warm = warm == 3 ? 3 : 0;
  o.halo = 1; o.p8 = 1; o.smap = 1;
  bf16_t* ix = tmp.get<bf16_t>((size_t)8 * 1024 * 640); bf16_t* iy = tmp.get<bf16_t>((size_t)8 * 1024 * 640); bf16_t* iw = tmp.get<bf16_t>((size_t)640 * 9 * 640);
  if (!ix || !iy || !iw) return -1;
  fill_rand(ix, (long long)8 * 1024 * 640, 11, 1.0f); fill_rand(iw, (long long)640 * 9 * 640, 12, 0.05f);
  WMat iwm; iwm.w = iw; iwm.N = 640; iwm.Cin = 640; iwm.Cpad = 640; iwm.taps = 9;
  GemmOpt io; io.bias = bias;
  hipEvent_t a, b; hipEventCreate(&a); hipEventCreate(&b);
  double tot = 0;
  for (int i = 0; i < iters + 1; ++i) {
    hipMemsetAsync(scratch, i, flush_bytes, 0);
    hipMemcpyAsync(x0, xs, xn * 2, hipMemcpyDeviceToDevice, 0);
    if (r) hipMemcpyAsync(y, r, (size_t)M * Nout * 2, hipMemcpyDeviceToDevice, 0);
    if (warm == 2 || warm >= 4) hipLaunchKernelGGL(touch_kernel, dim3(1024), dim3(256), 0, 0, (const u32x4*)w, (long long)(wn * 2 / 16), sink);
    for (int k = 0; k < (warm == 4 ? 1 : warm == 5 ? 2 : warm == 6 ? 4 : 0); ++k) CK(run_conv(nullptr, 0, ix, 640, nullptr, 0, 8, 32, 32, iwm, 3, iy, io, op_zero_page()));
    hipEventRecord(a, 0);
    if (warm == 1) hipLaunchKernelGGL(touch_kernel, dim3(1024), dim3(256), 0, 0, (const u32x4*)w, (long long)(wn * 2 / 16), sink);
    CK(run_conv(nullptr, 0, x0, C0, nullptr, 0, B, H, W, wm, ksize, y, o, op_zero_page()));
    hipEventRecord(b, 0); hipEventSynchronize(b);
    float t = 0; hipEventElapsedTime(&t, a, b);
    if (i > 0) tot += t;
  }
  *ms_out = tot / iters;
  hipEventDestroy(a); hipEventDestroy(b);
  return 0;
}

AGD_API int agd_bench_tblock(int kind, int B, int HW, int iters, double* ms_out) {
  Tmp tmp;
  const int C = (kind == 4 || kind == 5) ? 640 : 320, T = 77; const long long M = (long long)B * HW;
  if (kind == 4 || kind == 5) kind = kind == 4 ? 1 : 3;
  bf16_t* h = tmp.get<bf16_t>((size_t)M * C); bf16_t* o = tmp.get<bf16_t>((size_t)M * C);
  bf16_t* w1 = tmp.get<bf16_t>((size_t)8 * C * C); bf16_t* w1f = tmp.get<bf16_t>((size_t)8 * C * C);
  bf16_t* w2 = tmp.get<bf16_t>((size_t)4 * C * C); bf16_t* w2f = tmp.get<bf16_t>((size_t)4 * C * C);
  bf16_t* kv = tmp.get<bf16_t>((size_t)B * T * 2 * C);
  const int rslices = C == 640 ? 8 : 1;
  float* vec = tmp.get<float>((size_t)16 * C + 64); float* rec = tmp.get<float>((size_t)B * rslices * T * HW);
  if (!h || !o || !w1 || !w1f || !w2 || !w2f || !kv || !vec || !rec) return -1;
  fill_rand(h, M * C, 1, 1.0f); fill_rand(w1, 8LL * C * C, 2, 0.05f); fill_rand(w2, 4LL * C * C, 3, 0.03f); fill_rand(kv, (long long)B * T * 2 * C, 4, 1.0f);
  hipMemset(vec, 0, ((size_t)16 * C + 64) * 4); hipMemset(rec, 0, (size_t)B * rslices * T * HW * 4);
  FFusedP fp{}; AttnChainP ap{};
  if (kind == 0) {
    CK(launch_frag_order_w1(w1, w1f, C, 4 * C, 0)); CK(launch_frag_order_w(w2, w2f, C, 4 * C, C / 64, 128, 0));
    fp.h = h; fp.out = o; fp.w1f = w1f; fp.cs1 = vec; fp.b1 = vec + 8 * C; fp.w2f = w2f; fp.b2 = vec; fp.M = (int)M; fp.ln_eps = 1e-5f;
  } else {
    CK(launch_frag_order_w(w1, w1f, C, C, 5, C, 0)); CK(launch_frag_order_w(w2, w2f, C, C, 5, C, 0));
    ap.h = h; ap.out = o; ap.gamma = vec; ap.beta = vec; ap.ln_eps = 1e-5f; ap.wqf = w1f; ap.wof = w2f; ap.bo = vec; ap.kv = kv; ap.ldkv = 2 * C; ap.skv = (long long)T * 2 * C;
    ap.M = (int)M; ap.HW = HW; ap.T = T; ap.scale = 1.0f / sqrtf((float)(C / 8));
    ap.record = 1; ap.rec = rec; ap.rec_b0 = B / 2; ap.rec_T = T; ap.rec_hpb = 8 / rslices; ap.rec_head_stride = (long long)T * HW; ap.rec_img_stride = (long long)rslices * T * HW;
  }
  bf16_t* o2 = nullptr; float* cst = nullptr;
  if (kind == 2) {
    o2 = tmp.get<bf16_t>((size_t)M * C); cst = tmp.get<float>((size_t)(M / 128 + 1) * C * 2); if (!o2 || !cst) return -1;
    bf16_t* wpf = tmp.get<bf16_t>((size_t)C * C); if (!wpf) return -1;
    CK(launch_frag_order_w(w2, wpf, C, C, C / 64, C, 0));
    CK(launch_frag_order_w1(w1, w1f, C, 4 * C, 0)); CK(launch_frag_order_w(w2, w2f, C, 4 * C, C / 64, 128, 0));
    fp.h = h; fp.out = o; fp.w1f = w1f; fp.cs1 = vec; fp.b1 = vec + 8 * C; fp.w2f = w2f; fp.b2 = vec; fp.M = (int)M; fp.ln_eps = 1e-5f;
    fp.wpf = wpf; fp.bp = vec; fp.xres = o2; fp.pout = o; fp.colstat = cst;
  }
  if (kind == 3) {
    o2 = tmp.get<bf16_t>((size_t)M * C); bf16_t* wo1f = tmp.get<bf16_t>((size_t)C * C); if (!o2 || !wo1f) return -1;
    fill_rand(o2, M * C, 9, 1.0f);
    CK(launch_frag_order_w(w2, wo1f, C, C, 5, C, 0));
    ap.o1 = o2; ap.wo1f = wo1f; ap.bo1 = vec;
  }
  QkvChainP qp{};
  const bool qkvk = kind >= 6 && kind <= 9;
  if (qkvk) {
    bf16_t* qkv = tmp.get<bf16_t>((size_t)M * 3 * C); float* part = tmp.get<float>((size_t)B * (HW / 128) * C * 2); float* gv = tmp.get<float>((size_t)4 * C);
    if (!qkv || !part || !gv) return -1;
    hipMemset(part, 0x3C, (size_t)B * (HW / 128) * C * 2 * 4); hipMemset(gv, 0x3C, (size_t)4 * C * 4);
    CK(launch_frag_order_w(w2, w2f, C, C, 5, C, 0)); CK(launch_frag_order_w(w1, w1f, 3 * C, C, 5, C, 0));
    qp.x = h; qp.wbf = w2f; qp.wb_stride = 0; qp.rowadd = gv; qp.rowadd_stride = 0; qp.h = o; qp.gamma = gv + C; qp.beta = gv + 2 * C; qp.ln_eps = 1e-5f;
    qp.wqkvf = w1f; qp.qkv = qkv; qp.M = (int)M; qp.HW = HW; qp.rows64 = kind == 7 || kind == 9; qp.sched2 = kind >= 8;
    qp.gn_part = part; qp.gn_bm = 128; qp.gn_groups = 32; qp.gn_eps = 1e-6f; qp.gn_gamma = gv + 3 * C; qp.gn_beta = gv;
  }
  auto run = [&]() { return qkvk ? launch_qkv_chain(qp, C, 0) : (kind == 0 || kind == 2) ? launch_ff_fused(fp, C, 0) : launch_attn_chain(ap, C, 8, 0); };
  hipEvent_t a, b; hipEventCreate(&a); hipEventCreate(&b);
  for (int i = 0; i < 2; ++i) CK(run());
  hipEventRecord(a, 0);
  for (int i = 0; i < iters; ++i) CK(run());
  hipEventRecord(b, 0); hipEventSynchronize(b);
  float t = 0; hipEventElapsedTime(&t, a, b);
  *ms_out = t / iters;
  hipEventDestroy(a); hipEventDestroy(b);
  return 0;
}

AGD_API int agd_bench_attention(int B, int H, int D, int Nq, int Nk, int record, int iters, double* ms_out) {
  Tmp tmp;
  const int C = H * D;
  const bool self = (Nq == Nk);
  bf16_t* q = tmp.get<bf16_t>((size_t)B * Nq * (self ? 3 * C : C)); bf16_t* kv = self ? nullptr : tmp.get<bf16_t>((size_t)B * Nk * 2 * C);
  bf16_t* o = tmp.get<bf16_t>((size_t)B * Nq * C);
  float* rec = record ? tmp.get<float>((size_t)B * H * Nk * Nq) : nullptr;
  if (!q || !o || (!self && !kv) || (record && !rec)) return -1;
  fill_rand(q, (long long)B * Nq * (self ? 3 * C : C), 5, 1.0f); if (kv) fill_rand(kv, (long long)B * Nk * 2 * C, 6, 1.0f);
  if (rec) hipMemset(rec, 0, (size_t)B * H * Nk * Nq * 4);
  AttnP a{};
  if (self) { a.q = q; a.k = q + C; a.v = q + 2 * C; a.ldq = a.ldk = a.ldv = 3 * C; a.sq = a.sk = a.sv = (long long)Nq * 3 * C; }
  else { a.q = q; a.k = kv; a.v = kv + C; a.ldq = C; a.ldk = a.ldv = 2 * C; a.sq = (long long)Nq * C; a.sk = a.sv = (long long)Nk * 2 * C; }
  a.o = o; a.ldo = C; a.so = (long long)Nq * C; a.B = B; a.H = H; a.D = D; a.Nq = Nq; a.Nk = Nk; a.scale = 1.0f / sqrtf((float)D);
  if (record) { a.record_mode = record >= 2 ? 3 : 1; a.rec_hpb = record >= 2 ? (16 >> record < H ? 16 >> record : H) : 0; a.rec_b0 = B / 2; a.rec = rec;
                a.rec_T = Nk; a.rec_head_stride = (long long)Nk * Nq; a.rec_img_stride = a.rec_head_stride * (record >= 2 ? H / a.rec_hpb : H); }
  hipEvent_t e0, e1; hipEventCreate(&e0); hipEventCreate(&e1);
  for (int i = 0; i < 2; ++i) CK(launch_attention(a, 0));
  hipEventRecord(e0, 0);
  for (int i = 0; i < iters; ++i) CK(launch_attention(a, 0));
  hipEventRecord(e1, 0); hipEventSynchronize(e1);
  float t = 0; hipEventElapsedTime(&t, e0, e1);
  *ms_out = t / iters;
  hipEventDestroy(e0); hipEventDestroy(e1);
  return 0;
}

AGD_API int agd_bench_groupnorm_ex(int B, int HW, int C0, int C1, int fused_stats, int iters, double* ms_out) {
  Tmp tmp;
  const int C = C0 + C1;
  if (B < 1 || HW < 1 || C0 < 8 || C1 < 0 || iters < 1 || !ms_out) { agd_set_error("bench_groupnorm: bad arguments"); return -1; }
  bf16_t* x0 = tmp.get<bf16_t>((size_t)B * HW * C0); bf16_t* x1 = C1 ? tmp.get<bf16_t>((size_t)B * HW * C1) : nullptr;
  bf16_t* y = tmp.get<bf16_t>((size_t)B * HW * C);
  float* ws = tmp.get<float>((size_t)groupnorm_ws_floats(B, C, HW, 32)); float* g = tmp.get<float>(2 * C);
  if (!x0 || (C1 && !x1) || !y || !ws || !g) return -1;
  fill_rand(x0, (long long)B * HW * C0, 7, 1.0f); if (C1) fill_rand(x1, (long long)B * HW * C1, 8, 1.0f);
  hipMemset(g, 0, 2 * C * 4);
  GroupNormP p{}; p.x0 = x0; p.x1 = x1; p.C0 = C0; p.C1 = C1; p.y = y; p.gamma = g; p.beta = g + C; p.B = B; p.HW = HW; p.groups = 32; p.eps = 1e-5f; p.silu = 1; p.ws = ws;
  if (fused_stats) {
    if (HW % 128) { agd_set_error("bench_groupnorm: fused_stats needs HW %% 128 == 0"); return -1; }
    const size_t n0 = (size_t)B * (HW / 128) * C0 * 2, n1 = (size_t)B * (HW / 128) * C1 * 2;
    float* p0 = tmp.get<float>(n0); float* p1 = C1 ? tmp.get<float>(n1) : nullptr;
    if (!p0 || (C1 && !p1)) return -1;
    hipMemset(p0, 0, n0 * 4); if (C1) hipMemset(p1, 0, n1 * 4);
    p.part0 = p0; p.part1 = p1; p.bm0 = 128; p.bm1 = C1 ? 128 : 0;
  }
  hipEvent_t e0, e1; hipEventCreate(&e0); hipEventCreate(&e1);
  for (int i = 0; i < 2; ++i) CK(launch_groupnorm(p, 0));
  hipEventRecord(e0, 0);
  for (int i = 0; i < iters; ++i) CK(launch_groupnorm(p, 0));
  hipEventRecord(e1, 0); hipEventSynchronize(e1);
  float t = 0; hipEventElapsedTime(&t, e0, e1);
  *ms_out = t / iters;
// ... 1082 lines not shown
```

### agenda_amd/csrc/tblock.hip

```cpp
#include "kernels.h"
#include <type_traits>

typedef __attribute__((ext_vector_type(2))) float f32x2_t;
#ifdef AGD_EXPERIMENTS
int g_tb_variant = 0;
extern "C" __attribute__((visibility("default"))) void agd_set_tb_variant(int v) { g_tb_variant = v; }
#endif
#ifdef AGD_STAMPS
__device__ unsigned long long g_tb_ts[256];
__device__ int g_tb_ts_sel[2] = {-1, 0};
extern "C" __attribute__((visibility("default"))) int agd_tb_ts(int wg, int wave, unsigned long long* out) {
  if (out) return hipMemcpyFromSymbol(out, HIP_SYMBOL(g_tb_ts), 256 * 8) == hipSuccess ? 0 : -1;
  const int sel[2] = {wg, wave};
  return hipMemcpyToSymbol(HIP_SYMBOL(g_tb_ts_sel), sel, 8) == hipSuccess ? 0 : -1;
}
#define TB_TS_DECL const bool ts_on = (int)blockIdx.x == g_tb_ts_sel[0] && (int)threadIdx.x == g_tb_ts_sel[1] * 64; int ts_n = 0; if (ts_on) g_tb_ts[250] = __builtin_amdgcn_s_memrealtime();
#define TB_TS(k) do { if (ts_on && ts_n < 240) g_tb_ts[ts_n++] = ((unsigned long long)(k) << 56) | (__builtin_amdgcn_s_memtime() & 0x00FFFFFFFFFFFFFFull); } while (0)
#define TB_TS_END do { if (ts_on) { asm volatile("s_waitcnt vmcnt(0)" ::: "memory"); TB_TS(99); g_tb_ts[255] = ts_n; g_tb_ts[251] = __builtin_amdgcn_s_memrealtime(); } } while (0)
#else
#define TB_TS_DECL
#define TB_TS(k) do { } while (0)
#define TB_TS_END do { } while (0)
#endif

// ... 12 lines not shown
    *(u32x4*)(dst + idx * 8) = *(const u32x4*)(src + row * C + 32 * ks + 8 * g);
  }
}
__global__ __launch_bounds__(256) void frag_order_w_kernel(const bf16_t* __restrict__ src, bf16_t* __restrict__ dst, int N, int K, int NI, int KC) {
  const int NQ = N / (NI * 16), KSC = KC / 32, NCH = K / KC;
  const long long total = (long long)NCH * NQ * KSC * NI * 64;
  for (long long idx = (long long)blockIdx.x * 256 + threadIdx.x; idx < total; idx += (long long)gridDim.x * 256) {
    const int l = (int)(idx & 63); long long f = idx >> 6;
    const int j = (int)(f % NI); f /= NI;
    const int ks = (int)(f % KSC); f /= KSC;
    const int nq = (int)(f % NQ); const int c = (int)(f / NQ);
    const int rho = l & 15, g = l >> 4, qp = rho >> 2, rp = rho & 3;
    const long long n = (long long)nq * NI * 16 + qp * 4 * NI + 4 * j + rp;
    *(u32x4*)(dst + idx * 8) = *(const u32x4*)(src + n * K + (long long)c * KC + 32 * ks + 8 * g);
  }
}
int launch_frag_order_w1(const bf16_t* src, bf16_t* dst, int C, int HID, hipStream_t st) {
  if (C % 32 || HID % 128) { agd_set_error("frag_order_w1: C %d / hidden %d", C, HID); return -1; }
  hipLaunchKernelGGL(frag_order_w1_kernel, dim3(1024), dim3(256), 0, st, src, dst, C, HID);
  HIP_CHECK_RET(hipGetLastError());
  return 0;
}
int launch_frag_order_w(const bf16_t* src, bf16_t* dst, int N, int K, int NI, int KC, hipStream_t st) {
  if (N % (NI * 16) || K % KC || KC % 32) { agd_set_error("frag_order_w: N %d K %d NI %d KC %d", N, K, NI, KC); return -1; }
  hipLaunchKernelGGL(frag_order_w_kernel, dim3(1024), dim3(256), 0, st, src, dst, N, K, NI, KC);
  HIP_CHECK_RET(hipGetLastError());
  return 0;
}

#define TB_OOB 0x80000000u
template <int C> AGD_DEV int panel_swz(int ch, int row) {
  if constexpr ((C * 2) % 256 == 128) return (ch & ~7) | ((ch & 7) ^ ((row >> 1) & 7));
  else return (ch & ~15) | ((ch & 15) ^ (row & 15));
}
template <int C> struct XOff {
  static constexpr int XG = ((C * 2) % 256 == 128) ? 2 : 4;
  int xo[4];
  AGD_DEV XOff(int q, int px) {
#pragma unroll
    for (int t = 0; t < 4; ++t) xo[t] = ((C * 2) % 256 == 128) ? (((4 * (t & 1) + q) ^ ((px >> 1) & 7)) << 4) : (((4 * t + q) ^ px) << 4);
  }
  AGD_DEV int at(int ks) const { return (ks / XG) * (XG * 64) + xo[ks % XG]; }
};

template <int C, int BM = 128, int NW = 8>
AGD_DEV void panel_load_dma(const bf16_t* src, int m0, int M, char* panel, int wid, int lane) {
  constexpr int CHR = C / 8, PIECES = BM * CHR / 64;
  static_assert(PIECES % NW == 0, "pieces split evenly over the workgroup's waves");
#pragma unroll
  for (int i = 0; i < PIECES / NW; ++i) {
    const int piece = i * NW + wid, pos = piece * 64 + lane;
    const int row = pos / CHR, pc = pos - row * CHR;
    const int lc = panel_swz<C>(pc, row);
    const int m = m0 + row;
    const unsigned voff = m < M ? (unsigned)(((long long)m * C + lc * 8) * 2) : TB_OOB;
    bufdma16(src, panel + piece * 1024, voff, 0u);
  }
}

template <int C, int BM = 128>
AGD_DEV void panel_row_stats(const char* panel, float* lnst, int tid, float eps) {
  constexpr int CHR = C / 8, TPR = 512 / BM, PER = CHR / TPR;
  static_assert(CHR % TPR == 0, "chunks per row split over the row's threads");
  const int row = tid / TPR, part = tid % TPR;
  float S = 0.f, Q = 0.f;
#pragma unroll
  for (int cc = 0; cc < PER; ++cc) {
    const u32x4 v = *(const u32x4*)(panel + row * (C * 2) + panel_swz<C>(part * PER + cc, row) * 16);
#pragma unroll
    for (int e = 0; e < 4; ++e) {
      const float a = __uint_as_float(v[e] << 16), b = __uint_as_float(v[e] & 0xFFFF0000u);
      S += a + b; Q += a * a + b * b;
    }
  }
#pragma unroll
  for (int o = 1; o < TPR; o <<= 1) { S += __shfl_xor(S, o); Q += __shfl_xor(Q, o); }
  if (part == 0) {
    const float mu = S * (1.0f / C);
    float var = Q * (1.0f / C) - mu * mu; var = var < 0.f ? 0.f : var;
    *(f32x2_t*)(lnst + row * 2) = f32x2_t{mu, rsqrtf(var + eps)};
  }
}

typedef u32x4 __attribute__((aligned(8))) u32x4_a8;
template <int NI> AGD_DEV void load_row_chunk(const bf16_t* p, u32x2 (&r)[NI]) {
#pragma unroll
  for (int t = 0; t + 1 < NI; t += 2) { const u32x4 v = *(const u32x4_a8*)(p + 4 * t); r[t] = u32x2{v[0], v[1]}; r[t + 1] = u32x2{v[2], v[3]}; }
  if (NI & 1) r[NI - 1] = *(const u32x2*)(p + 4 * (NI - 1));
}
template <int NI> AGD_DEV void store_row_chunk(bf16_t* p, const u32x2 (&r)[NI]) {
#pragma unroll
  for (int t = 0; t + 1 < NI; t += 2) *(u32x4_a8*)(p + 4 * t) = u32x4{r[t][0], r[t][1], r[t + 1][0], r[t + 1][1]};
  if (NI & 1) *(u32x2*)(p + 4 * (NI - 1)) = r[NI - 1];
}

#define TB_F 10
#define TB_D 8
template <int C>
AGD_DEV void panel_gemm_head(u32x4 (&ring)[TB_F], const bf16_t* wf, unsigned wbase, unsigned lane16, unsigned wbytes = C * C * 2) {
  const auto wrs = __builtin_amdgcn_make_buffer_rsrc((void*)wf, 0, wbytes, 0x00020000);
#pragma unroll
  for (int f = 0; f < TB_D; ++f) ring[f % TB_F] = __builtin_bit_cast(u32x4, __builtin_amdgcn_raw_buffer_load_b128(wrs, lane16, wbase + (unsigned)f * 1024u, 0));
}
struct TbNoHook { AGD_DEV void operator()() const {} };
template <int C, bool ZERO = true, int MI = 4, class Late = TbNoHook>
AGD_DEV void panel_gemm_body(u32x4 (&ring)[TB_F], f32x4 (&acc)[MI][5], const bf16_t* wf, unsigned wbase, unsigned lane16, const char* xrow, const XOff<C>& xo,
                             unsigned wbytes = C * C * 2, Late&& late = Late()) {
  constexpr int NI = 5, KS = C / 32, NFR = KS * NI, PITCH = C * 2;
  const auto wrs = __builtin_amdgcn_make_buffer_rsrc((void*)wf, 0, wbytes, 0x00020000);
  if constexpr (ZERO) {
#pragma unroll
  for (int i = 0; i < MI; ++i)
#pragma unroll
    for (int j = 0; j < NI; ++j) acc[i][j] = f32x4{0.f, 0.f, 0.f, 0.f};
  }
  bf16x8 xf[MI];
#pragma unroll
  for (int f = 0; f < NFR; ++f) {
    if (f + TB_D < NFR) ring[(f + TB_D) % TB_F] = __builtin_bit_cast(u32x4, __builtin_amdgcn_raw_buffer_load_b128(wrs, lane16, wbase + (unsigned)(f + TB_D) * 1024u, 0));
    if (f == NFR - TB_D) late();
    __builtin_amdgcn_sched_barrier(0);
    if (f % NI == 0) {
      const int ks = f / NI;
#pragma unroll
      for (int i = 0; i < MI; ++i) xf[i] = *(const bf16x8*)(xrow + i * 16 * PITCH + xo.at(ks));
    }
#pragma unroll
    for (int i = 0; i < MI; ++i)
      acc[i][f % NI] = __builtin_amdgcn_mfma_f32_16x16x32_bf16(__builtin_bit_cast(bf16x8, ring[f % TB_F]), xf[i], acc[i][f % NI], 0, 0, 0);
  }
}

template <int C, int VAR = 0, int POST = 0>
__global__ __launch_bounds__(512, 2) void ff_fused_kernel(const FFusedP p) {
  constexpr int BM = 128, HID = 4 * C, HC = 128, NCH = HID / HC, KS1 = C / 32, KS2 = HC / 32, NI2 = C / 64;
  constexpr int PITCH = C * 2;
  static_assert(C % 64 == 0 && (C / 8) % 8 == 0 && KS1 % 2 == 0, "panel geometry");
  extern __shared__ __attribute__((aligned(16))) char smem[];
  char* panel = smem;
  char* hbuf = smem + BM * PITCH;
  float* lnst = (float*)(hbuf + 2 * BM * HC * 2);
  float* cbufs = lnst + BM * 2;

  const int tid = threadIdx.x, lane = tid & 63;
  const int wid = __builtin_amdgcn_readfirstlane(tid >> 6);
  const int mh = wid >> 2, nq = wid & 3;
  const int m0 = blockIdx.x * BM;
  TB_TS_DECL
  TB_TS(1);

  panel_load_dma<C>(p.h, m0, p.M, panel, wid, lane);
  asm volatile("s_waitcnt vmcnt(0)" ::: "memory");
  __syncthreads();
  panel_row_stats<C>(panel, lnst, tid, p.ln_eps);
  { const auto cs1r0 = __builtin_amdgcn_make_buffer_rsrc((void*)p.cs1, 0, (unsigned)(2 * HID * 4), 0x00020000);
    const auto b1r0 = __builtin_amdgcn_make_buffer_rsrc((void*)p.b1, 0, (unsigned)(2 * HID * 4), 0x00020000);
    const unsigned off = (unsigned)((((tid >> 7) & 1) ? HID : 0) + (tid & (HC - 1))) * 4u;
    ((float*)(hbuf + 2 * BM * HC * 2) + BM * 2)[tid] = __builtin_bit_cast(float, wid < 4 ? __builtin_amdgcn_raw_buffer_load_b32(cs1r0, off, 0, 0) : __builtin_amdgcn_raw_buffer_load_b32(b1r0, off, 0, 0)); }
  __syncthreads();

  f32x4 acc2[4][NI2];
#pragma unroll
  for (int i = 0; i < 4; ++i)
#pragma unroll
    for (int j = 0; j < NI2; ++j) acc2[i][j] = f32x4{0.f, 0.f, 0.f, 0.f};
  f32x4 acc1[4][4];

  const auto w1rs = __builtin_amdgcn_make_buffer_rsrc((void*)p.w1f, 0, (unsigned)(2 * HID * C * 2), 0x00020000);
  const auto w2rs = __builtin_amdgcn_make_buffer_rsrc((void*)p.w2f, 0, (unsigned)(HID * C * 2), 0x00020000);
#define ldw1(sbase, f) __builtin_bit_cast(u32x4, __builtin_amdgcn_raw_buffer_load_b128(w1rs, lane16, (sbase) + (unsigned)(f) * 1024u, 0))
#define ldw2(sbase, f) __builtin_bit_cast(u32x4, __builtin_amdgcn_raw_buffer_load_b128(w2rs, lane16, (sbase) + (unsigned)(f) * 1024u, 0))
  constexpr bool NOW = (VAR & 2) != 0, NOX = (VAR & 4) != 0;

  constexpr int F = TB_F, D = TB_D, DX = 2, N2 = KS2 * NI2, N1 = KS1 * 4;
  static_assert((N1 + N2) % F == 0 && D < F && D <= N2 && DX <= D, "ring geometry");
  u32x4 ring[F];

  auto lane_now = [&]() __attribute__((always_inline)) { int l = lane; asm volatile("" : "+v"(l)); return l; };
  auto gemm2 = [&](int c, bool pre, bool has_next, unsigned nexts) __attribute__((always_inline)) {
    const int l_ = lane_now(), q = l_ >> 4, px = l_ & 15;
    const unsigned lane16 = (unsigned)l_ * 16u;
    const char* hb = hbuf + (c & 1) * (BM * HC * 2) + (64 * mh + px) * (HC * 2);
    const unsigned wp = __builtin_amdgcn_readfirstlane((unsigned)(((c * 4 + nq) * KS2) * NI2) * 1024u);
    if (!pre && !NOW) {
#pragma unroll
      for (int f = 0; f < DX; ++f) ring[f % F] = ldw2(wp, f);
    }
    if constexpr (!NOW) {
#pragma unroll
      for (int f = DX; f < D; ++f) ring[f % F] = ldw2(wp, f);
    }
    bf16x8 hf[4];
#pragma unroll
    for (int f = 0; f < N2; ++f) {
      const int tgt = f + D;
      if constexpr (!NOW) {
        if (tgt < N2) ring[tgt % F] = ldw2(wp, tgt);
        else if (has_next) ring[tgt % F] = ldw1(nexts, tgt - N2);
      }
      __builtin_amdgcn_sched_barrier(0);
      if (f % NI2 == 0 && (!NOX || f == 0)) {
#pragma unroll
        for (int i = 0; i < 4; ++i) hf[i] = *(const bf16x8*)(hb + i * 16 * (HC * 2) + (((4 * (f / NI2) + q) ^ px) << 4));
      }
#pragma unroll
      for (int i = 0; i < 4; ++i)
        acc2[i][f % NI2] = __builtin_amdgcn_mfma_f32_16x16x32_bf16(__builtin_bit_cast(bf16x8, ring[f % F]), hf[i], acc2[i][f % NI2], 0, 0, 0);
    }
  };

  auto gemm1 = [&](int c, bool pre, bool has_next, unsigned nexts) __attribute__((always_inline)) {
#pragma unroll
    for (int i = 0; i < 4; ++i)
#pragma unroll
      for (int j = 0; j < 4; ++j) acc1[i][j] = f32x4{0.f, 0.f, 0.f, 0.f};
    const unsigned wp = __builtin_amdgcn_readfirstlane((unsigned)(((c * 4 + nq) * KS1) * 4) * 1024u);
    const int l_ = lane_now(), q = l_ >> 4, px = l_ & 15;
    const unsigned lane16 = (unsigned)l_ * 16u;
    const int sx = (px >> 1) & 7;
    const int xoff0 = ((q ^ sx) << 4), xoff1 = (((4 + q) ^ sx) << 4);
    const char* xrow = panel + (64 * mh + px) * PITCH;
    if (!pre && !NOW) {
#pragma unroll
      for (int f = 0; f < D; ++f) ring[(N2 + f) % F] = ldw1(wp, f);
    }
    bf16x8 xf[4];
#pragma unroll
    for (int f = 0; f < N1; ++f) {
      const int tgt = f + D;
      if constexpr (!NOW) {
        if (tgt < N1) ring[(N2 + tgt) % F] = ldw1(wp, tgt);
        else if (has_next && tgt - N1 < DX) ring[(N2 + tgt) % F] = ldw2(nexts, tgt - N1);
      }
      __builtin_amdgcn_sched_barrier(0);
      if (f % 4 == 0 && (!NOX || f == 0)) {
        const int ks = f / 4;
#pragma unroll
        for (int i = 0; i < 4; ++i) xf[i] = *(const bf16x8*)(xrow + i * 16 * PITCH + (ks >> 1) * 128 + ((ks & 1) ? xoff1 : xoff0));
      }
#pragma unroll
      for (int i = 0; i < 4; ++i)
        acc1[i][f % 4] = __builtin_amdgcn_mfma_f32_16x16x32_bf16(__builtin_bit_cast(bf16x8, ring[(N2 + f) % F]), xf[i], acc1[i][f % 4], 0, 0, 0);
    }
  };

  const auto cs1rs = __builtin_amdgcn_make_buffer_rsrc((void*)p.cs1, 0, (unsigned)(2 * HID * 4), 0x00020000);
  const auto b1rs = __builtin_amdgcn_make_buffer_rsrc((void*)p.b1, 0, (unsigned)(2 * HID * 4), 0x00020000);
  auto cload = [&](int c) __attribute__((always_inline)) {
    const unsigned off = (unsigned)((((tid >> 7) & 1) ? HID : 0) + HC * c + (tid & (HC - 1))) * 4u;
    return __builtin_bit_cast(float, wid < 4 ? __builtin_amdgcn_raw_buffer_load_b32(cs1rs, off, 0, 0) : __builtin_amdgcn_raw_buffer_load_b32(b1rs, off, 0, 0));
  };
  auto cstore = [&](int c, float v) __attribute__((always_inline)) { cbufs[(c % 3) * (4 * HC) + tid] = v; };
  static_assert(HC == 128, "one float per thread and chunk");
  auto geglu = [&](int c) __attribute__((always_inline)) {
    const int l_ = lane_now(), q = l_ >> 4, px = l_ & 15;
    const int rbase = 64 * mh + px;
    const float* cb = cbufs + (c % 3) * (4 * HC) + 32 * nq + 8 * q;
    char* hb = hbuf + (c & 1) * (BM * HC * 2);
    float mu[4], rs[4];
#pragma unroll
    for (int i = 0; i < 4; ++i) { const f32x2_t v = *(const f32x2_t*)(lnst + (rbase + 16 * i) * 2); mu[i] = v[0]; rs[i] = v[1]; }
#pragma unroll
    for (int t = 0; t < 2; ++t) {
      const f32x4 csv = *(const f32x4*)(cb + 4 * t), csg = *(const f32x4*)(cb + HC + 4 * t), bv = *(const f32x4*)(cb + 2 * HC + 4 * t), bg = *(const f32x4*)(cb + 3 * HC + 4 * t);
#pragma unroll
      for (int i = 0; i < 4; ++i) {
        float o[4];
#pragma unroll
        for (int r = 0; r < 4; ++r) {
          const float v = rs[i] * (acc1[i][t][r] - mu[i] * csv[r]) + bv[r];
          const float g = rs[i] * (acc1[i][2 + t][r] - mu[i] * csg[r]) + bg[r];
          o[r] = (VAR & 1) ? v + g : v * gelu_erf_f(g);
        }
        *(u32x2*)(hb + (rbase + 16 * i) * (HC * 2) + (((4 * nq + q) ^ px) << 4) + 8 * t) = u32x2{pack_bf2(o[0], o[1]), pack_bf2(o[2], o[3])};
      }
    }
  };

  bool pre2 = false;
  if constexpr (NOW) {
    const unsigned lane16 = (unsigned)lane * 16u;
#pragma unroll
    for (int f = 0; f < F; ++f) ring[f] = ldw1(0u, f);
  }
  auto interval = [&](int k) __attribute__((always_inline)) {
    const bool cn = k + 1 < NCH;
    float cv = 0.f;
    if (cn) cv = cload(k + 1);
    if (!(VAR & 8) && mh == 1 && k >= 1 && k <= NCH) geglu(k - 1);
    const int c2 = k - 1 - mh, c2n = k - mh;
    const bool v2 = c2 >= 0 && c2 < NCH, v1 = k < NCH, v2n = c2n >= 0 && c2n < NCH;
    const unsigned w1s = __builtin_amdgcn_readfirstlane((unsigned)(((k * 4 + nq) * KS1) * 4) * 1024u);
    const unsigned w2ns = __builtin_amdgcn_readfirstlane((unsigned)(((c2n * 4 + nq) * KS2) * NI2) * 1024u);
    if (v2) gemm2(c2, pre2, v1, w1s);
    if (v1) gemm1(k, v2, v2n, w2ns);
    pre2 = v1 && v2n;
    if (!(VAR & 8) && mh == 0 && k < NCH) geglu(k);
    if (cn) cstore(k + 1, cv);
    if (k <= NCH) __syncthreads();
  };
  static_assert(NCH >= 4, "steady intervals");
  TB_TS(2);
#pragma unroll 1
  for (int k = 0; k < 2; ++k) interval(k);
  TB_TS(3);
  if (mh == 0) {
    for (int k = 2; k < NCH; ++k) {
      const unsigned w1s = __builtin_amdgcn_readfirstlane((unsigned)(((k * 4 + nq) * KS1) * 4) * 1024u);
      const unsigned w2ns = __builtin_amdgcn_readfirstlane((unsigned)(((k * 4 + nq) * KS2) * NI2) * 1024u);
      const bool cn = k + 1 < NCH;
      float cv = 0.f;
      if (cn) cv = cload(k + 1);
      gemm2(k - 1, true, true, w1s);
      TB_TS(10);
      gemm1(k, true, true, w2ns);
      TB_TS(11);
      if (!(VAR & 8)) geglu(k);
      TB_TS(12);
      if (cn) cstore(k + 1, cv);
      __syncthreads();
      TB_TS(13);
    }
  } else {
    for (int k = 2; k < NCH; ++k) {
      const bool cn = k + 1 < NCH;
      float cv = 0.f;
      if (cn) cv = cload(k + 1);
      if (!(VAR & 8)) geglu(k - 1);
      TB_TS(12);
      const unsigned w1s = __builtin_amdgcn_readfirstlane((unsigned)(((k * 4 + nq) * KS1) * 4) * 1024u);
      const unsigned w2ns = __builtin_amdgcn_readfirstlane((unsigned)((((k - 1) * 4 + nq) * KS2) * NI2) * 1024u);
      gemm2(k - 2, true, true, w1s);
      TB_TS(10);
      gemm1(k, true, true, w2ns);
      TB_TS(11);
      if (cn) cstore(k + 1, cv);
      __syncthreads();
      TB_TS(13);
    }
  }
  TB_TS(4);
  pre2 = true;
#pragma unroll 1
  for (int k = NCH; k <= NCH + 1; ++k) interval(k);
  TB_TS(5);

  const int l_e = lane_now(), q = l_e >> 4, px = l_e & 15;
  const int rbase = 64 * mh + px;
  const unsigned lane16 = (unsigned)l_e * 16u;
  const char* xrow = panel + rbase * PITCH;
  const int ncol0 = (C / 4) * nq + 4 * NI2 * q;
  constexpr bool post = POST != 0;
  constexpr bool premul = POST == 2;
  static_assert(F == TB_F, "the proj_out stage reuses the weight ring");
  const unsigned pwbase = __builtin_amdgcn_readfirstlane((unsigned)(nq * KS1 * NI2) * 1024u);
  if (post) panel_gemm_head<C>(ring, p.wpf, pwbase, lane16);
  if constexpr (!premul) {
  float b2v[NI2 * 4];
#pragma unroll
  for (int t = 0; t < NI2; ++t) *(f32x4*)&b2v[4 * t] = *(const f32x4*)(p.b2 + ncol0 + 4 * t);
#pragma unroll
  for (int i = 0; i < 4; ++i) {
    const int row = rbase + 16 * i, m = m0 + row;
    if (!post && m >= p.M) continue;
    u32x2 pk[NI2];
#pragma unroll
    for (int t = 0; t < NI2; ++t) {
      const int n = ncol0 + 4 * t;
      char* pa = panel + row * PITCH + panel_swz<C>(n >> 3, row) * 16 + (n & 7) * 2;
      const u32x2 r = *(const u32x2*)pa;
      pk[t][0] = pack_bf2(acc2[i][t][0] + b2v[4 * t] + __uint_as_float(r[0] << 16), acc2[i][t][1] + b2v[4 * t + 1] + __uint_as_float(r[0] & 0xFFFF0000u));
      pk[t][1] = pack_bf2(acc2[i][t][2] + b2v[4 * t + 2] + __uint_as_float(r[1] << 16), acc2[i][t][3] + b2v[4 * t + 3] + __uint_as_float(r[1] & 0xFFFF0000u));
      if (post) *(u32x2*)pa = pk[t];
    }
    if (!post) store_row_chunk<NI2>(p.out + (long long)m * C + ncol0, pk);
  }
  }
  if constexpr (post) {
  if constexpr (!premul) __syncthreads();
  u32x2 xr[4][NI2];
  auto ld_xr = [&]() __attribute__((always_inline)) {
#pragma unroll
    for (int i = 0; i < 4; ++i) { const int m = m0 + rbase + 16 * i, ms = m < p.M ? (p.xres_rows > 0 ? m % p.xres_rows : m) : 0; load_row_chunk<NI2>(p.xres + (long long)ms * C + ncol0, xr[i]); }
  };
  ld_xr();
  panel_gemm_body<C, !premul>(ring, acc2, p.wpf, pwbase, lane16, xrow, XOff<C>(q, px));
  float bpv[NI2 * 4];
#pragma unroll
  for (int t = 0; t < NI2; ++t) *(f32x4*)&bpv[4 * t] = *(const f32x4*)(p.bp + ncol0 + 4 * t);
  float cs[NI2 * 4], cq[NI2 * 4];
#pragma unroll
  for (int e = 0; e < NI2 * 4; ++e) { cs[e] = 0.f; cq[e] = 0.f; }
#pragma unroll
  for (int i = 0; i < 4; ++i) {
    const int m = m0 + rbase + 16 * i;
    const bool live = m < p.M;
    const long long mo = (long long)(live ? m : 0) * C + ncol0;
    u32x2 pkk[NI2];
#pragma unroll
    for (int t = 0; t < NI2; ++t) {
      u32x2 pk;
      pk[0] = pack_bf2(acc2[i][t][0] + bpv[4 * t] + __uint_as_float(xr[i][t][0] << 16), acc2[i][t][1] + bpv[4 * t + 1] + __uint_as_float(xr[i][t][0] & 0xFFFF0000u));
      pk[1] = pack_bf2(acc2[i][t][2] + bpv[4 * t + 2] + __uint_as_float(xr[i][t][1] << 16), acc2[i][t][3] + bpv[4 * t + 3] + __uint_as_float(xr[i][t][1] & 0xFFFF0000u));
      pkk[t] = pk;
      if (live) {
        const float a0 = __uint_as_float(pk[0] << 16), a1 = __uint_as_float(pk[0] & 0xFFFF0000u), a2 = __uint_as_float(pk[1] << 16), a3 = __uint_as_float(pk[1] & 0xFFFF0000u);
        cs[4 * t] += a0; cs[4 * t + 1] += a1; cs[4 * t + 2] += a2; cs[4 * t + 3] += a3;
        cq[4 * t] += a0 * a0; cq[4 * t + 1] += a1 * a1; cq[4 * t + 2] += a2 * a2; cq[4 * t + 3] += a3 * a3;
      }
    }
    if (live) store_row_chunk<NI2>(p.pout + mo, pkk);
  }
  if (p.colstat) {
#pragma unroll
    for (int e = 0; e < NI2 * 4; ++e) {
#pragma unroll
      for (int o = 1; o < 16; o <<= 1) { cs[e] += __shfl_xor(cs[e], o); cq[e] += __shfl_xor(cq[e], o); }
    }
    float* stg = (float*)hbuf;
    if (px == 0) {
#pragma unroll
      for (int e = 0; e < NI2 * 4; ++e) { stg[(mh * C + ncol0 + e) * 2] = cs[e]; stg[(mh * C + ncol0 + e) * 2 + 1] = cq[e]; }
    }
    __syncthreads();
    if (tid < C) {
      float* op = p.colstat + ((long long)blockIdx.x * C + tid) * 2;
      op[0] = stg[tid * 2] + stg[(C + tid) * 2]; op[1] = stg[tid * 2 + 1] + stg[(C + tid) * 2 + 1];
    }
  }
  }
  TB_TS_END;
}

int launch_ff_fused(const FFusedP& p, int C, hipStream_t st) {
  if (C != 320) { agd_set_error("ff_fused: C = %d is not built (320 only)", C); return -1; }
  if (p.M < 1 || !p.h || !p.out || !p.w1f || !p.w2f || !p.cs1 || !p.b1 || !p.b2) { agd_set_error("ff_fused: bad arguments"); return -1; }
  if ((long long)p.M * C * 2 >= (1LL << 31)) { agd_set_error("ff_fused: activation too large for 32-bit offsets"); return -1; }
  constexpr int lds = 128 * 320 * 2 + 2 * 128 * 128 * 2 + 128 * 8 + 3 * 4 * 128 * 4;
  const void* kfn = p.wpf ? (p.premul ? (const void*)ff_fused_kernel<320, 0, 2> : (const void*)ff_fused_kernel<320, 0, 1>) : (const void*)ff_fused_kernel<320>;
  if (p.wpf && (!p.bp || !p.xres || !p.pout)) { agd_set_error("ff_fused: the proj_out stage needs bias, residual and output"); return -1; }
  if (p.premul && !p.wpf) { agd_set_error("ff_fused: the pre-multiplied form is the proj_out stage's"); return -1; }
#ifdef AGD_EXPERIMENTS
  static const void* const vars[16] = {(const void*)ff_fused_kernel<320, 0>, (const void*)ff_fused_kernel<320, 1>, (const void*)ff_fused_kernel<320, 2>, (const void*)ff_fused_kernel<320, 3>,
                                       (const void*)ff_fused_kernel<320, 4>, nullptr, (const void*)ff_fused_kernel<320, 6>, (const void*)ff_fused_kernel<320, 7>,
                                       (const void*)ff_fused_kernel<320, 8>, nullptr, (const void*)ff_fused_kernel<320, 10>, nullptr, nullptr, nullptr, (const void*)ff_fused_kernel<320, 14>, nullptr};
  if (!p.wpf && g_tb_variant > 0 && g_tb_variant < 16 && vars[g_tb_variant]) kfn = vars[g_tb_variant];
#endif
  int dev = 0; HIP_CHECK_RET(hipGetDevice(&dev));
  if (dev < 0 || dev >= AGD_MAX_DEVICES) { agd_set_error("ff_fused: device ordinal %d out of range", dev); return -1; }
  HIP_CHECK_RET(hipFuncSetAttribute(kfn, hipFuncAttributeMaxDynamicSharedMemorySize, lds));
  FFusedP pp = p;
  void* args[] = {&pp};
  HIP_CHECK_RET(hipLaunchKernel(kfn, dim3((p.M + 127) / 128), dim3(512), args, lds, st));
  return 0;
}

template <int C, int PRE, int MI = 4>
__global__ __launch_bounds__(512, 2) void attn_chain_kernel(const AttnChainP p) {
  TB_TS_DECL
  TB_TS(0);
  constexpr int NQ = C / 80, MH = 8 / NQ, BM = 16 * MI * MH, QBN = BM / 32;
  static_assert(MI == 4 || (MI == 2 && C == 640), "32-row panels: C = 640 only");
  constexpr int H = 8, D = C / H, KS = C / 32, NI = 5, PITCH = C * 2, CHR = C / 8;
  static_assert(C == 320 || C == 640, "8 heads of 40 / 80");
  constexpr int KB = 3, KEYS = 96, KSTEPS = (D + 15) / 16, DBLK = (D + 31) / 32, CH = D / 8;
  constexpr int KPITCH = ((2 * KSTEPS) | 1) * 16, VPITCH = (DBLK | 1) * 64;
  constexpr int KVSTAGE = KEYS * (KPITCH + VPITCH);
  constexpr int NCHUNK = KEYS * CH, LD_IT = (NCHUNK + 255) / 256;
  extern __shared__ __attribute__((aligned(16))) char smem[];
  char* panel = smem;
  char* kvs = smem + BM * PITCH;
  float* lnst = (float*)(kvs + 2 * KVSTAGE);
  float* pst = lnst + BM * 2;
  float* gbs = pst + NQ * BM * 2;

  const int tid = threadIdx.x, lane = tid & 63;
  const int wid = __builtin_amdgcn_readfirstlane(tid >> 6);
  const int mh = wid / NQ, nq = wid % NQ;
  const int q = lane >> 4, px = lane & 15;
  const int qb = wid & (QBN - 1), hhalf = wid >> 2;
  const bool attn_wave = QBN == 4 || (wid & 3) < QBN;
  const int c = lane & 31, hh = lane >> 5;
  const int m0 = blockIdx.x * BM;
  const int b = m0 / p.HW, pix0 = m0 - b * p.HW;
  const int m0s = p.src_rows > 0 ? m0 % p.src_rows : m0;
  TB_TS(1);
  const int gbi = tid < C / 2 ? tid : 0;
  const f32x4 gbv = *(const f32x4*)((gbi < C / 4 ? p.gamma : p.beta - C) + 4 * gbi);
  panel_load_dma<C, BM>(PRE ? p.o1 : p.h, m0s, p.src_rows > 0 ? p.src_rows : p.M, panel, wid, lane);
  TB_TS(40);

  char* sK = kvs + hhalf * KVSTAGE;
  char* sV = sK + KEYS * KPITCH;
  const int t4 = tid & 255;
  constexpr int KPADC = KPITCH / 16 - CH;
  for (int i = t4; i < KEYS * KPADC; i += 256) { const int r = i / KPADC, cc = CH + i % KPADC; *(u32x4*)(sK + r * KPITCH + cc * 16) = u32x4{0, 0, 0, 0}; }
  TB_TS(41);
  u32x4 kreg[LD_IT], vreg[LD_IT];
  unsigned kvoff[LD_IT];
#pragma unroll
  for (int it = 0; it < LD_IT; ++it) {
    const int idx = t4 + it * 256, r = idx / CH, cc = idx - r * CH;
    kvoff[it] = idx < NCHUNK ? (unsigned)((r * p.ldkv + cc * 8) * 2) : TB_OOB;
  }
  const unsigned kv_bytes = (unsigned)(((long long)(p.T - 1) * p.ldkv + D) * 2);
  const bf16_t* kvb = p.kv + (long long)b * p.skv;
  auto kv_load = [&](int h) {
    const auto krs = __builtin_amdgcn_make_buffer_rsrc((void*)(kvb + h * D), 0, kv_bytes, 0x00020000);
    const auto vrs = __builtin_amdgcn_make_buffer_rsrc((void*)(kvb + C + h * D), 0, kv_bytes, 0x00020000);
#pragma unroll
    for (int it = 0; it < LD_IT; ++it) {
      kreg[it] = __builtin_bit_cast(u32x4, __builtin_amdgcn_raw_buffer_load_b128(krs, kvoff[it], 0, 0));
      vreg[it] = __builtin_bit_cast(u32x4, __builtin_amdgcn_raw_buffer_load_b128(vrs, kvoff[it], 0, 0));
    }
  };
  auto kv_store = [&]() {
#pragma unroll
    for (int it = 0; it < LD_IT; ++it) {
      const int idx = t4 + it * 256, r = idx / CH, cc = idx - r * CH;
      if (idx < NCHUNK) { *(u32x4*)(sK + r * KPITCH + cc * 16) = kreg[it]; *(u32x4*)(sV + r * VPITCH + cc * 16) = vreg[it]; }
    }
  };
  kv_load(4 * hhalf);
  TB_TS(42);
// ... 767 lines not shown
```

### agenda_amd/ops.py

```python
from __future__ import annotations

import torch

from . import _lib


def _f32c(t):
    assert t.is_cuda, "ops run on the GPU only (no CPU fallback)"
    return t.detach().to(torch.float32).contiguous()


_P8 = {0: 0, 1: 2, 2: 4, 3: 8}


def conv2d(x, w, bias=None, stride=1, padding=None, upsample=False, halo=False, p8=0, smap=False, phases=False, pc=0, xcd_block=False):
    lib = _lib.load()
    x, w = _f32c(x), _f32c(w)
    b = _f32c(bias) if bias is not None else None
    B, Cin, H, W = x.shape
    Cout, _, k, _ = w.shape
    pad = (1 if k == 3 else 0) if padding is None else padding
    up = 2 if upsample else 1
    Ho = (H * up + 2 * pad - k) // stride + 1
    Wo = (W * up + 2 * pad - k) // stride + 1
    y = torch.empty(B, Cout, Ho, Wo, device=x.device, dtype=torch.float32)
    _lib.check(lib.agd_op_conv2d_ex(_lib.ptr(x), _lib.ptr(w), _lib.ptr(b), _lib.ptr(y), B, Cin, H, W, Cout, k, stride,
                                    pad, int(upsample), (1 if halo else 0) | _P8[p8] | (16 if smap else 0) | (64 if phases else 0) | ((int(pc) & 15) << 7) | ((int(pc) & 48) << 8) | (2048 if xcd_block else 0), _lib.current_stream_ptr()), None, "agd_op_conv2d")
    return y


def linear(x, w, bias=None, residual=None, geglu=False, p8=0, wreg=False, kgroups=False, pc=0, xcd_block=False):
    lib = _lib.load()
    x2 = _f32c(x).reshape(-1, x.shape[-1])
    w = _f32c(w)
    M, K = x2.shape
    N = w.shape[0]
    Nout = N // 2 if geglu else N
    b = _f32c(bias) if bias is not None else None
    r = _f32c(residual).reshape(M, Nout) if residual is not None else None
    y = torch.empty(M, Nout, device=x.device, dtype=torch.float32)
    _lib.check(lib.agd_op_linear(_lib.ptr(x2), _lib.ptr(w), _lib.ptr(b), _lib.ptr(r), _lib.ptr(y), M, K, N, int(geglu) | _P8[p8] | (16 if wreg else 0) | (32 if kgroups else 0) | (64 if (wreg and kgroups) else 0) | ((int(pc) & 15) << 7) | ((int(pc) & 48) << 8) | (2048 if xcd_block else 0),
                                 _lib.current_stream_ptr()), None, "agd_op_linear")
    return y.reshape(*x.shape[:-1], Nout)


def group_norm(x, groups, gamma, beta, eps=1e-5, silu=False):
    lib = _lib.load()
    x = _f32c(x)
    B, Cc = x.shape[:2]
    HW = x[0, 0].numel()
    y = torch.empty_like(x)
    _lib.check(lib.agd_op_groupnorm(_lib.ptr(x), _lib.ptr(_f32c(gamma)), _lib.ptr(_f32c(beta)), _lib.ptr(y), B, Cc, HW,
                                    groups, float(eps), int(silu), _lib.current_stream_ptr()), None, "agd_op_groupnorm")
    return y


def layer_norm(x, gamma, beta, eps=1e-5):
    lib = _lib.load()
    x = _f32c(x)
    Cc = x.shape[-1]
    rows = x.numel() // Cc
    y = torch.empty_like(x)
    _lib.check(lib.agd_op_layernorm(_lib.ptr(x), _lib.ptr(_f32c(gamma)), _lib.ptr(_f32c(beta)), _lib.ptr(y), rows, Cc,
                                    float(eps), _lib.current_stream_ptr()), None, "agd_op_layernorm")
    return y


def ff_fused(x, gamma, beta, w1, b1, w2, b2, eps=1e-5):
    lib = _lib.load()
    Cc = x.shape[-1]
    x2 = _f32c(x).reshape(-1, Cc)
    y = torch.empty_like(x2)
    _lib.check(lib.agd_op_ff_fused(_lib.ptr(x2), _lib.ptr(_f32c(gamma)), _lib.ptr(_f32c(beta)), _lib.ptr(_f32c(w1)), _lib.ptr(_f32c(b1)),
                                   _lib.ptr(_f32c(w2)), _lib.ptr(_f32c(b2)), _lib.ptr(y), x2.shape[0], Cc, float(eps),
                                   _lib.current_stream_ptr()), None, "agd_op_ff_fused")
    return y.reshape(x.shape)


def attn_chain(x, gamma, beta, wq, kv, wo, bo, heads=8, eps=1e-5, return_probs=False, rows32=False):
    lib = _lib.load()
    x, kv = _f32c(x), _f32c(kv)
    B, HW, Cc = x.shape
    T = kv.shape[1]
    y = torch.empty_like(x)
    pr = torch.empty(B, T, HW, device=x.device, dtype=torch.float32) if return_probs else None
    _lib.check(lib.agd_op_attn_chain(_lib.ptr(x), _lib.ptr(_f32c(gamma)), _lib.ptr(_f32c(beta)), _lib.ptr(_f32c(wq)), _lib.ptr(kv), _lib.ptr(_f32c(wo)),
                                     _lib.ptr(_f32c(bo)), _lib.ptr(y), _lib.ptr(pr), B, HW, T, Cc, heads | (256 if rows32 else 0), float(eps), _lib.current_stream_ptr()),
               None, "agd_op_attn_chain")
    return (y, pr) if return_probs else y


def xattn_premul(x, gamma, beta, wq, kv, wo, bo, heads=8, eps=1e-5, return_probs=False):
    lib = _lib.load()
    x, kv = _f32c(x), _f32c(kv)
    B, HW, Cc = x.shape
    T = kv.shape[1]
    y = torch.empty_like(x)
    pr = torch.empty(B, heads, T, HW, device=x.device, dtype=torch.float32) if return_probs else None
    _lib.check(lib.agd_op_xattn_premul(_lib.ptr(x), _lib.ptr(_f32c(gamma)), _lib.ptr(_f32c(beta)), _lib.ptr(_f32c(wq)), _lib.ptr(kv), _lib.ptr(_f32c(wo)),
                                       _lib.ptr(_f32c(bo)), _lib.ptr(y), _lib.ptr(pr), B, HW, T, Cc, heads, float(eps), _lib.current_stream_ptr()),
               None, "agd_op_xattn_premul")
    return (y, pr) if return_probs else y


def attention(q, k, v, heads, scale=None, return_probs=False):
    lib = _lib.load()
    q, k, v = _f32c(q), _f32c(k), _f32c(v)
    B, Nq, Cc = q.shape
    Nk = k.shape[1]
    D = Cc // heads
    scale = D ** -0.5 if scale is None else scale
    o = torch.empty_like(q)
    probs = torch.empty(B, heads, Nk, Nq, device=q.device, dtype=torch.float32) if return_probs else None
    _lib.check(lib.agd_op_attention(_lib.ptr(q), _lib.ptr(k), _lib.ptr(v), _lib.ptr(o), B, heads, D, Nq, Nk, float(scale),
                                    _lib.ptr(probs), _lib.current_stream_ptr()), None, "agd_op_attention")
    return (o, probs) if return_probs else o


def attention_headsum(q, k, v, heads, scale=None):
    lib = _lib.load()
    q, k, v = _f32c(q), _f32c(k), _f32c(v)
    B, Nq, Cc = q.shape
    Nk = k.shape[1]
    D = Cc // heads
    scale = D ** -0.5 if scale is None else scale
    o = torch.empty_like(q)
    probs = torch.empty(B, Nk, Nq, device=q.device, dtype=torch.float32)
    _lib.check(lib.agd_op_attention_headsum(_lib.ptr(q), _lib.ptr(k), _lib.ptr(v), _lib.ptr(o), B, heads, D, Nq, Nk, float(scale),
                                            _lib.ptr(probs), _lib.current_stream_ptr()), None, "agd_op_attention_headsum")
    return o, probs


def bicubic_clamp_mean(maps, out_side):
    lib = _lib.load()
    maps = _f32c(maps)
    n, T, side, _ = maps.shape
    out = torch.empty(T, out_side, out_side, device=maps.device, dtype=torch.float32)
    _lib.check(lib.agd_op_bicubic_clamp_mean(_lib.ptr(maps), n, T, side, out_side, _lib.ptr(out),
                                             _lib.current_stream_ptr()), None, "agd_op_bicubic_clamp_mean")
    return out


def attn_reg_loss(attn_map: torch.Tensor, obj_idx, fg_idx, bg_idx, coef: float, want_grad: bool = True):
    lib = _lib.load()
    m = attn_map.detach().to(torch.float32).contiguous()
    assert m.is_cuda and m.ndim == 4
    B, T = m.shape[:2]
    P = m.shape[2] * m.shape[3]
    host = [torch.as_tensor(list(map(int, i)) if not torch.is_tensor(i) else i.detach().cpu(), dtype=torch.int32) for i in (obj_idx, fg_idx, bg_idx)]
    has = host[0] >= 0
    if bool(has.any()):
        worst = max(int(h[has].max()) for h in host)
        if worst >= T:
            raise IndexError(f"index {worst} is out of bounds for dimension 0 with size {T}")
    idx = [h.to(m.device).contiguous() for h in host]
    loss = torch.empty(B, 2, device=m.device, dtype=torch.float32)
    dmap = torch.empty_like(m) if want_grad else None
    _lib.check(lib.agd_op_attn_reg_loss(_lib.ptr(m), B, T, P, _lib.ptr(idx[0]), _lib.ptr(idx[1]), _lib.ptr(idx[2]), float(coef), _lib.ptr(loss),
                                        _lib.ptr(dmap), _lib.current_stream_ptr()), None, "agd_op_attn_reg_loss")
# ... 52 lines not shown
```

### include/agenda_hip.h

```cpp
#ifndef AGENDA_HIP_H
#define AGENDA_HIP_H
#ifdef __cplusplus
extern "C" {
#endif

typedef struct agd_ctx agd_ctx;

#define AGD_MAX_LEVELS 8

typedef struct agd_config {
  int struct_size;
  int in_channels, out_channels, n_levels;
  int block_out_channels[AGD_MAX_LEVELS];
  int down_cross[AGD_MAX_LEVELS];
  int num_heads[AGD_MAX_LEVELS];
  int layers_per_block, cross_attention_dim, use_linear_projection, norm_num_groups;
  int vae_latent_channels, vae_out_channels, vae_n_levels;
  int vae_block_out_channels[AGD_MAX_LEVELS];
  int vae_layers_per_block, vae_norm_num_groups;
  float vae_scaling_factor;
  int max_tokens;
  int prediction_type;
  long long workspace_bytes;
  int text_hidden, text_layers, text_heads, text_intermediate, text_vocab, text_max_pos;
// ... 88 lines not shown
int agd_image_embeds(agd_ctx* ctx, const unsigned char* images, int batch, int h, int w, float* out, void* stream);

typedef struct agd_gligen_config {
  int struct_size;
  int max_objs;
  int positive_len;
  int fourier_freqs;
} agd_gligen_config;
int agd_gligen_configure(agd_ctx* ctx, const agd_gligen_config* gcfg);
int agd_gligen_set(agd_ctx* ctx, const float* boxes, const float* pos_emb, const float* masks, int batch2, void* stream);
int agd_gligen_set_schedule(agd_ctx* ctx, const int* flags, int n);
int agd_gligen_clear(agd_ctx* ctx);
int agd_gligen_objs(agd_ctx* ctx, float* out);
int agd_gligen_fuser(agd_ctx* ctx, const char* block_name, const float* x, int batch2, int h, int w, float* out, void* stream);

int agd_unet_forward(agd_ctx* ctx, const float* sample, int batch2, int latent_side, float timestep, float* out,
                     void* stream);
int agd_unet_forward_hw(agd_ctx* ctx, const float* sample, int batch2, int latent_h, int latent_w, float timestep, float* out, void* stream);
int agd_unet_forward_ts(agd_ctx* ctx, const float* sample, int batch2, int latent_side, const float* timesteps, float* out, void* stream);
int agd_unet_forward_ts_hw(agd_ctx* ctx, const float* sample, int batch2, int latent_h, int latent_w, const float* timesteps, float* out,
                           void* stream);

int agd_cfg_ddim_step(agd_ctx* ctx, const float* eps, float* latents, int batch, int latent_side, float guidance,
                      float alpha_t, float alpha_prev, void* stream);
int agd_cfg_ddim_step_hw(agd_ctx* ctx, const float* eps, float* latents, int batch, int latent_h, int latent_w, float guidance,
                         float alpha_t, float alpha_prev, void* stream);

int agd_denoise(agd_ctx* ctx, float* latents, int batch, int latent_side, int n_steps, const float* timesteps,
                const float* alpha_t, const float* alpha_prev, float guidance, void* stream);
int agd_denoise_hw(agd_ctx* ctx, float* latents, int batch, int latent_h, int latent_w, int n_steps, const float* timesteps,
                   const float* alpha_t, const float* alpha_prev, float guidance, void* stream);

int agd_denoise_plms(agd_ctx* ctx, float* latents, int batch, int latent_side, int n_evals, const float* timesteps,
                     const float* sample_coeff, const float* eps_coeff, float guidance, void* stream);
int agd_denoise_plms_hw(agd_ctx* ctx, float* latents, int batch, int latent_h, int latent_w, int n_evals, const float* timesteps,
                        const float* sample_coeff, const float* eps_coeff, float guidance, void* stream);

int agd_denoise_dpm(agd_ctx* ctx, float* latents, int batch, int latent_side, int n_evals, const float* timesteps,
                    const float* coeffs, float guidance, void* stream);
int agd_denoise_dpm_hw(agd_ctx* ctx, float* latents, int batch, int latent_h, int latent_w, int n_evals, const float* timesteps,
                       const float* coeffs, float guidance, void* stream);

int agd_vae_decode(agd_ctx* ctx, const float* latents, int batch, int latent_side, unsigned char* out_u8,
                   float* out_f32, void* stream);
int agd_vae_decode_hw(agd_ctx* ctx, const float* latents, int batch, int latent_h, int latent_w, unsigned char* out_u8,
                      float* out_f32, void* stream);

int agd_vae_encode(agd_ctx* ctx, const float* image, int batch, int side, float* mean_out, float* logvar_out, void* stream);
int agd_vae_encode_hw(agd_ctx* ctx, const float* image, int batch, int h, int w, float* mean_out, float* logvar_out, void* stream);

int agd_set_option(agd_ctx* ctx, const char* name, int value);

int agd_record_config(agd_ctx* ctx, int mode, int is_train, int rec_tokens);
int agd_record_reset(agd_ctx* ctx, int batch, int latent_side, void* stream);
int agd_record_reset_hw(agd_ctx* ctx, int batch, int latent_h, int latent_w, void* stream);
int agd_daam_global(agd_ctx* ctx, int img, int rows, float* out, void* stream);
int agd_hook_global(agd_ctx* ctx, float* out, void* stream);
int agd_hook_count(agd_ctx* ctx);
int agd_hook_last_map(agd_ctx* ctx, float* out, int n_query, void* stream);

int agd_attn_processor(agd_ctx* ctx, const char* layer, const float* hidden, const float* ctx_emb, const float* attn_mask,
                       int batch2, int n_query, int tokens, float* out, int record, void* stream);
int agd_cross_attn(agd_ctx* ctx, const char* layer, const float* hidden, const float* ctx_emb, int batch2,
                   int n_query, int tokens, float* out, int record, void* stream);

int agd_hook_reset(agd_ctx* ctx, int rows, int latent_side, void* stream);
int agd_hook_num_maps(agd_ctx* ctx);
int agd_hook_map_dims(agd_ctx* ctx, int k, int* dims3);
int agd_hook_map(agd_ctx* ctx, int k, float* out, void* stream);
int agd_op_attn_reg_loss(const float* map, int B, int T, int P, const int* obj_idx, const int* fg_idx, const int* bg_idx, float coef,
                         float* loss_out, float* dmap, void* stream);
int agd_attn_processor_backward(agd_ctx* ctx, const char* layer, const float* hidden, const float* ctx_emb, const float* d_out,
                                const float* d_map, int is_train, int batch2, int n_query, int tokens, float* d_hidden, float* d_ctx,
                                void* stream);

int agd_op_conv2d(const float* x_nchw, const float* w, const float* bias, float* y_nchw, int B, int Cin, int H, int W,
                  int Cout, int ksize, int stride, int pad, int upsample, void* stream);
int agd_op_conv2d_ex(const float* x, const float* w, const float* bias, float* y, int B, int Cin, int H, int W, int Cout,
                     int ksize, int stride, int pad, int upsample, int flags, void* stream);
int agd_op_linear(const float* x, const float* w, const float* bias, const float* residual, float* y, int M, int K,
                  int N, int geglu, void* stream);
int agd_op_ff_fused(const float* x, const float* gamma, const float* beta, const float* w1, const float* b1, const float* w2,
                    const float* b2, float* y, int M, int C, float eps, void* stream);
int agd_op_attn_chain(const float* x, const float* gamma, const float* beta, const float* wq, const float* kv, const float* wo,
                      const float* bo, float* y, float* probs_sum, int B, int HW, int T, int C, int heads, float eps, void* stream);
int agd_op_xattn_premul(const float* x, const float* gamma, const float* beta, const float* wq, const float* kv, const float* wo,
                        const float* bo, float* y, float* probs, int B, int HW, int T, int C, int heads, float eps, void* stream);
int agd_op_groupnorm(const float* x_nchw, const float* gamma, const float* beta, float* y_nchw, int B, int C, int HW,
                     int groups, float eps, int silu, void* stream);
int agd_op_conv_groupnorm(const float* x_nchw, const float* w, const float* bias, const float* gamma, const float* beta, float* y_nchw,
                          int B, int Cin, int H, int W, int Cout, int groups, float eps, int silu, int fused, void* stream);
int agd_op_layernorm(const float* x, const float* gamma, const float* beta, float* y, int rows, int C, float eps,
                     void* stream);
int agd_op_attention(const float* q, const float* k, const float* v, float* o, int B, int H, int D, int Nq, int Nk,
                     float scale, float* probs_out, void* stream);
int agd_op_attention_headsum(const float* q, const float* k, const float* v, float* o, int B, int H, int D, int Nq, int Nk,
                             float scale, float* probs_sum_out, void* stream);
int agd_op_bicubic_clamp_mean(const float* maps, int n_maps, int T, int side, int S, float* out, void* stream);

int agd_op_heatmap_u8(const float* hm, int n, int npix, unsigned char* out, void* stream);
int agd_op_resize_u8_pil(const unsigned char* in, int n, int H, int W, int C, int oh, int ow, unsigned char* out, void* stream);
int agd_op_stack_heatmaps(const unsigned char* obj, const unsigned char* fg, const unsigned char* bg, long long npix,
                          unsigned char* rgb, unsigned char* inv, void* stream);

int agd_lora_add(agd_ctx* ctx, const char* target_key, const float* down, const float* up, int rank, float alpha);
int agd_lora_set_scale(agd_ctx* ctx, float s, void* stream);
int agd_lora_clear(agd_ctx* ctx);
int agd_lora_count(agd_ctx* ctx);
float agd_lora_scale(agd_ctx* ctx);

int agd_op_window_gather(const float* canvas, float* views, int B, int C, int Lh, int Lw, int window, int stride, int v0, int n, void* stream);
int agd_op_window_mean(const float* views, float* canvas, int B, int C, int Lh, int Lw, int window, int stride, void* stream);
int agd_denoise_panorama(agd_ctx* ctx, float* canvas, int batch, int Lh, int Lw, int window, int stride, int view_batch, int n_steps,
                         const float* timesteps, const float* alpha_t, const float* alpha_prev, float guidance, void* stream);
int agd_daam_global_panorama(agd_ctx* ctx, int img, int rows, float* out, void* stream);

int agd_freeu_set(agd_ctx* ctx, float s1, float s2, float b1, float b2);
int agd_freeu_clear(agd_ctx* ctx);
int agd_freeu_counts(agd_ctx* ctx, long long* counts);
int agd_op_freeu(const float* hidden_nchw, const float* skip_nchw, float* hidden_out, float* skip_out, int B, int Ch, int Cs, int H, int W,
                 float b, float s, void* stream);

#define AGD_N_CLASSES 11
int agd_profile_begin(agd_ctx* ctx);
int agd_profile_end(agd_ctx* ctx, double* ms, double* flops, long long* launches);
int agd_profile_end_ex(agd_ctx* ctx, double mfma_peak_flops, double hbm_peak_bytes, double* ms, double* flops, double* bytes,
                       double* roof_ms, double* roof_ms_hbm_bound, long long* launches);
const char* agd_profile_class_name(int cls);

#ifdef AGD_EXPERIMENTS
int agd_bench_conv(int B, int H, int W, int C0, int C1, int Cout, int ksize, int stride, int up, int geglu, int with_residual,
                   int iters, double* ms_out);
int agd_bench_attention(int B, int H, int D, int Nq, int Nk, int record, int iters, double* ms_out);
int agd_bench_conv_cold(int B, int H, int W, int C0, int Cout, int ksize, int geglu, int with_residual, int warm, int iters, double* ms_out);
int agd_bench_groupnorm(int B, int HW, int C, int iters, double* ms_out);
int agd_bench_groupnorm_ex(int B, int HW, int C0, int C1, int fused_stats, int iters, double* ms_out);
#endif

const char* agd_version(void);

#ifdef __cplusplus
}
#endif
#endif
```

Before: 9.009.

## Add rescheduled FF-fused premul kernel overlapping weight prefetch with panel load

Adds a second schedule for the fused feed-forward plus proj_out kernel at C=320, and turns it on by default through a new TBF_FF_SCHED2 flag. The new schedule prefetches the first weight tiles before the activation panel DMA and splits the two half-block waves into staggered GEMM1/GEMM2 pipelines. It also streams the proj_out weights into the ring during the final GEMM2, so the separate proj head load goes away. Column-stat reductions switch from shuffles to DPP row sums. A standalone test entry point is added as well; the risk is extra register pressure and schedule-correctness bugs in the hand-pipelined code.

Result: no change. 9.082, median of 6 (+0.8%).

```diff
diff --git a/agenda_amd/_lib.py b/agenda_amd/_lib.py
--- a/agenda_amd/_lib.py
+++ b/agenda_amd/_lib.py
@@ -172,6 +172,7 @@
     "agd_op_conv_groupnorm": (C.c_int, [_P] * 6 + [C.c_int] * 6 + [C.c_float, C.c_int, C.c_int, _P]),
     "agd_op_layernorm": (C.c_int, [_P, _P, _P, _P, C.c_int, C.c_int, C.c_float, _P]),
     "agd_op_ff_fused": (C.c_int, [_P] * 8 + [C.c_int, C.c_int, C.c_float, _P]),
+    "agd_op_ff_fused_proj": (C.c_int, [_P] * 11 + [C.c_int, C.c_int, C.c_int, C.c_float, C.c_int, _P]),
     "agd_op_attn_chain": (C.c_int, [_P] * 9 + [C.c_int] * 5 + [C.c_float, _P]),
     "agd_op_xattn_premul": (C.c_int, [_P] * 9 + [C.c_int] * 5 + [C.c_float, _P]),
     "agd_op_attention": (C.c_int, [_P, _P, _P, _P, C.c_int, C.c_int, C.c_int, C.c_int, C.c_int, C.c_float, _P, _P]),
diff --git a/agenda_amd/csrc/kernels.h b/agenda_amd/csrc/kernels.h
--- a/agenda_amd/csrc/kernels.h
+++ b/agenda_amd/csrc/kernels.h
@@ -76,6 +76,7 @@
   const bf16_t* wpf; const float* bp; const bf16_t* xres; bf16_t* pout; float* colstat;
   int xres_rows;
   int premul;
+  int sched2;
 };
 int launch_ff_fused(const FFusedP& p, int C, hipStream_t st);
 struct AttnChainP {
diff --git a/agenda_amd/csrc/model.hip b/agenda_amd/csrc/model.hip
--- a/agenda_amd/csrc/model.hip
+++ b/agenda_amd/csrc/model.hip
@@ -92,7 +92,8 @@
   TBF_ATTN2_ROWS32  = 1 << 10,
   TBF_QKV_ROWS64    = 1 << 11,
   TBF_QKV_SCHED2    = 1 << 12,
-  TBF_DEFAULT       = 0x1fff & ~TBF_QKV_640,
+  TBF_FF_SCHED2     = 1 << 13,
+  TBF_DEFAULT       = 0x3fff & ~TBF_QKV_640,
 };
 
 struct ProfEv { int cls; double flops, bytes; hipEvent_t a, b; };
@@ -576,7 +577,7 @@
   XLayer* xl;
   TbAttn2 attn2; int chain_rows32;
   bool daam;
-  TbFf ff;
+  TbFf ff; int ff_sched2;
   bool wreg_proj;
   bool stats_head, stats_attn1, stats_attn2;
   bool stats_ipa;
@@ -650,6 +651,7 @@
   if (ff_fused) {
     const bool proj = tb(TBF_FF_PROJ) && has(pre + "proj_out.frag");
     p.ff = !proj ? FF_FUSED : tb(TBF_FF_PREMUL) && has(t + "ff.w2p.frag") ? FF_FUSED_PREMUL : FF_FUSED_PROJ;
+    p.ff_sched2 = p.ff == FF_FUSED_PREMUL && tb(TBF_FF_SCHED2);
   } else p.ff = c->opt_ffproj && has(pre + "ffproj.weight") ? FF_FFPROJ : FF_PLAIN;
   auto itx = c->xl_idx.find(t + "attn2");
   p.xl = itx == c->xl_idx.end() ? nullptr : &c->xl[itx->second];
@@ -861,7 +863,7 @@
     fp.wpf = fpw->w; fp.bp = bp; fp.xres = s.xres; fp.pout = out.p;
     if (p.ff == FF_FUSED_PREMUL) {
       GETW(f2p, t + "ff.w2p.frag"); GETV(bcp, s.pre + "ffproj.bias");
-      fp.w2f = f2p->w; fp.bp = bcp; fp.premul = 1;
+      fp.w2f = f2p->w; fp.bp = bcp; fp.premul = 1; fp.sched2 = p.ff_sched2;
     }
     if (p.dup == DUP_LAZY) fp.xres_rows = s.Mshared;
     out.cpart_bm = 0;
@@ -2781,6 +2783,35 @@
   return 0;
 }
 
+AGD_API int agd_op_ff_fused_proj(const float* x, const float* gamma, const float* beta, const float* w1, const float* b1, const float* w2p, const float* bpp, const float* wp,
+                                 const float* xres, float* y, float* colstat, int M, int C, int xres_rows, float eps, int sched2, void* stream) {
+  hipStream_t st = S(stream); Tmp tmp;
+  if (C != 320) { agd_set_error("op_ff_fused_proj: C = %d (320 only)", C); return -1; }
+  if (xres_rows < 1 || xres_rows > M) { agd_set_error("op_ff_fused_proj: %d residual rows for M = %d", xres_rows, M); return -1; }
+  const int H8 = 8 * C, H4 = 4 * C;
+  bf16_t* xb = tmp.get<bf16_t>((size_t)M * C); bf16_t* yb = tmp.get<bf16_t>((size_t)M * C); bf16_t* rb = tmp.get<bf16_t>((size_t)xres_rows * C);
+  bf16_t* w1b = tmp.get<bf16_t>((size_t)H8 * C); bf16_t* w1l = tmp.get<bf16_t>((size_t)H8 * C); bf16_t* w1f = tmp.get<bf16_t>((size_t)H8 * C);
+  bf16_t* w2b = tmp.get<bf16_t>((size_t)C * H4); bf16_t* w2f = tmp.get<bf16_t>((size_t)C * H4);
+  bf16_t* wpb = tmp.get<bf16_t>((size_t)C * C); bf16_t* wpf = tmp.get<bf16_t>((size_t)C * C);
+  float* cs = tmp.get<float>(H8); float* bf = tmp.get<float>(H8);
+  if (!xb || !yb || !rb || !w1b || !w1l || !w1f || !w2b || !w2f || !wpb || !wpf || !cs || !bf) return -1;
+  CK(launch_f32_to_bf16(x, xb, (long long)M * C, st));
+  CK(launch_f32_to_bf16(xres, rb, (long long)xres_rows * C, st));
+  CK(launch_convert_weight(w1, w1b, H8, C, 1, C, 16, st));
+  CK(launch_ln_fold_weight(w1b, gamma, beta, b1, H8, C, 16, w1l, cs, bf, st));
+  CK(launch_frag_order_w1(w1l, w1f, C, H4, st));
+  CK(launch_convert_weight(w2p, w2b, C, H4, 1, H4, 0, st));
+  CK(launch_frag_order_w(w2b, w2f, C, H4, C / 64, 128, st));
+  CK(launch_convert_weight(wp, wpb, C, C, 1, C, 0, st));
+  CK(launch_frag_order_w(wpb, wpf, C, C, C / 64, C, st));
+  FFusedP fp{}; fp.h = xb; fp.out = xb; fp.w1f = w1f; fp.cs1 = cs; fp.b1 = bf; fp.w2f = w2f; fp.b2 = bpp; fp.M = M; fp.ln_eps = eps;
+  fp.wpf = wpf; fp.bp = bpp; fp.xres = rb; fp.pout = yb; fp.colstat = colstat; fp.xres_rows = xres_rows < M ? xres_rows : 0; fp.premul = 1; fp.sched2 = sched2 ? 1 : 0;
+  CK(launch_ff_fused(fp, C, st));
+  CK(launch_bf16_to_f32(yb, y, (long long)M * C, st));
+  hipStreamSynchronize(st);
+  return 0;
+}
+
 AGD_API int agd_op_attn_chain(const float* x, const float* gamma, const float* beta, const float* wq, const float* kv, const float* wo,
                               const float* bo, float* y, float* probs_sum, int B, int HW, int T, int C, int heads, float eps, void* stream) {
   hipStream_t st = S(stream); Tmp tmp;
@@ -3017,6 +3048,8 @@
   Tmp tmp;
   const int C = (kind == 4 || kind == 5) ? 640 : 320, T = 77; const long long M = (long long)B * HW;
   if (kind == 4 || kind == 5) kind = kind == 4 ? 1 : 3;
+  const int ffpre = kind == 10 || kind == 11 ? kind - 9 : 0;
+  if (ffpre) kind = 2;
   bf16_t* h = tmp.get<bf16_t>((size_t)M * C); bf16_t* o = tmp.get<bf16_t>((size_t)M * C);
   bf16_t* w1 = tmp.get<bf16_t>((size_t)8 * C * C); bf16_t* w1f = tmp.get<bf16_t>((size_t)8 * C * C);
   bf16_t* w2 = tmp.get<bf16_t>((size_t)4 * C * C); bf16_t* w2f = tmp.get<bf16_t>((size_t)4 * C * C);
@@ -3043,7 +3076,7 @@
     CK(launch_frag_order_w(w2, wpf, C, C, C / 64, C, 0));
     CK(launch_frag_order_w1(w1, w1f, C, 4 * C, 0)); CK(launch_frag_order_w(w2, w2f, C, 4 * C, C / 64, 128, 0));
     fp.h = h; fp.out = o; fp.w1f = w1f; fp.cs1 = vec; fp.b1 = vec + 8 * C; fp.w2f = w2f; fp.b2 = vec; fp.M = (int)M; fp.ln_eps = 1e-5f;
-    fp.wpf = wpf; fp.bp = vec; fp.xres = o2; fp.pout = o; fp.colstat = cst;
+    fp.wpf = wpf; fp.bp = vec; fp.xres = o2; fp.pout = o; fp.colstat = cst; fp.premul = ffpre != 0; fp.sched2 = ffpre == 2;
   }
   if (kind == 3) {
     o2 = tmp.get<bf16_t>((size_t)M * C); bf16_t* wo1f = tmp.get<bf16_t>((size_t)C * C); if (!o2 || !wo1f) return -1;
diff --git a/agenda_amd/csrc/tblock.hip b/agenda_amd/csrc/tblock.hip
--- a/agenda_amd/csrc/tblock.hip
+++ b/agenda_amd/csrc/tblock.hip
@@ -118,6 +118,17 @@
   }
 }
 
+template <int CTRL> AGD_DEV float dpp_mov_f(float v) {
+  return __builtin_bit_cast(float, __builtin_amdgcn_update_dpp(0, __builtin_bit_cast(int, v), CTRL, 0xF, 0xF, false));
+}
+AGD_DEV float row16_sum_dpp(float v) {
+  v += dpp_mov_f<0xB1>(v);
+  v += dpp_mov_f<0x4E>(v);
+  v += dpp_mov_f<0x141>(v);
+  v += dpp_mov_f<0x140>(v);
+  return v;
+}
+
 typedef u32x4 __attribute__((aligned(8))) u32x4_a8;
 template <int NI> AGD_DEV void load_row_chunk(const bf16_t* p, u32x2 (&r)[NI]) {
 #pragma unroll
@@ -167,8 +178,9 @@
   }
 }
 
-template <int C, int VAR = 0, int POST = 0>
+template <int C, int VAR = 0, int POST = 0, int SCHED = 0>
 __global__ __launch_bounds__(512, 2) void ff_fused_kernel(const FFusedP p) {
+  static_assert(SCHED == 0 || (POST == 2 && VAR == 0), "the round-7 schedule is built for the production form");
   constexpr int BM = 128, HID = 4 * C, HC = 128, NCH = HID / HC, KS1 = C / 32, KS2 = HC / 32, NI2 = C / 64;
   constexpr int PITCH = C * 2;
   static_assert(C % 64 == 0 && (C / 8) % 8 == 0 && KS1 % 2 == 0, "panel geometry");
@@ -185,15 +197,20 @@
   TB_TS_DECL
   TB_TS(1);
 
+  if constexpr (SCHED == 0) {
   panel_load_dma<C>(p.h, m0, p.M, panel, wid, lane);
   asm volatile("s_waitcnt vmcnt(0)" ::: "memory");
   __syncthreads();
+  TB_TS(20);
   panel_row_stats<C>(panel, lnst, tid, p.ln_eps);
+  TB_TS(21);
   { const auto cs1r0 = __builtin_amdgcn_make_buffer_rsrc((void*)p.cs1, 0, (unsigned)(2 * HID * 4), 0x00020000);
     const auto b1r0 = __builtin_amdgcn_make_buffer_rsrc((void*)p.b1, 0, (unsigned)(2 * HID * 4), 0x00020000);
     const unsigned off = (unsigned)((((tid >> 7) & 1) ? HID : 0) + (tid & (HC - 1))) * 4u;
     ((float*)(hbuf + 2 * BM * HC * 2) + BM * 2)[tid] = __builtin_bit_cast(float, wid < 4 ? __builtin_amdgcn_raw_buffer_load_b32(cs1r0, off, 0, 0) : __builtin_amdgcn_raw_buffer_load_b32(b1r0, off, 0, 0)); }
   __syncthreads();
+  TB_TS(22);
+  }
 
   f32x4 acc2[4][NI2];
 #pragma unroll
@@ -213,7 +230,9 @@
   u32x4 ring[F];
 
   auto lane_now = [&]() __attribute__((always_inline)) { int l = lane; asm volatile("" : "+v"(l)); return l; };
-  auto gemm2 = [&](int c, bool pre, bool has_next, unsigned nexts) __attribute__((always_inline)) {
+  static_assert(SCHED == 0 || N2 % F == 0, "a stream that follows GEMM2 starts at ring slot 0");
+  const auto wprs = __builtin_amdgcn_make_buffer_rsrc((void*)p.wpf, 0, (unsigned)(C * C * 2), 0x00020000);
+  auto gemm2 = [&](int c, bool pre, int nk, unsigned nexts, bool pre_all = false) __attribute__((always_inline)) {
     const int l_ = lane_now(), q = l_ >> 4, px = l_ & 15;
     const unsigned lane16 = (unsigned)l_ * 16u;
     const char* hb = hbuf + (c & 1) * (BM * HC * 2) + (64 * mh + px) * (HC * 2);
@@ -223,8 +242,10 @@
       for (int f = 0; f < DX; ++f) ring[f % F] = ldw2(wp, f);
     }
     if constexpr (!NOW) {
+      if (!(SCHED && pre_all)) {
 #pragma unroll
       for (int f = DX; f < D; ++f) ring[f % F] = ldw2(wp, f);
+      }
     }
     bf16x8 hf[4];
 #pragma unroll
@@ -232,7 +253,11 @@
       const int tgt = f + D;
       if constexpr (!NOW) {
         if (tgt < N2) ring[tgt % F] = ldw2(wp, tgt);
-        else if (has_next) ring[tgt % F] = ldw1(nexts, tgt - N2);
+        else if (nk == 1) ring[tgt % F] = ldw1(nexts, tgt - N2);
+        else if constexpr (SCHED != 0) {
+          if (nk == 2) ring[tgt % F] = ldw2(nexts, tgt - N2);
+          else if (nk == 3) ring[tgt % F] = __builtin_bit_cast(u32x4, __builtin_amdgcn_raw_buffer_load_b128(wprs, lane16, nexts + (unsigned)(tgt - N2) * 1024u, 0));
+        }
       }
       __builtin_amdgcn_sched_barrier(0);
       if (f % NI2 == 0 && (!NOX || f == 0)) {
@@ -245,7 +270,8 @@
     }
   };
 
-  auto gemm1 = [&](int c, bool pre, bool has_next, unsigned nexts) __attribute__((always_inline)) {
+  const auto nrs0 = __builtin_amdgcn_make_buffer_rsrc(mh ? (void*)p.w1f : (void*)p.w2f, 0, (unsigned)((mh ? 2 : 1) * HID * C * 2), 0x00020000);
+  auto gemm1 = [&](int c, bool pre, bool has_next, unsigned nexts, int pre_n = 0, bool next_sel = false) __attribute__((always_inline)) {
 #pragma unroll
     for (int i = 0; i < 4; ++i)
 #pragma unroll
@@ -258,7 +284,7 @@
     const char* xrow = panel + (64 * mh + px) * PITCH;
     if (!pre && !NOW) {
 #pragma unroll
-      for (int f = 0; f < D; ++f) ring[(N2 + f) % F] = ldw1(wp, f);
+      for (int f = 0; f < D; ++f) if (SCHED == 0 || f >= pre_n) ring[(N2 + f) % F] = ldw1(wp, f);
     }
     bf16x8 xf[4];
 #pragma unroll
@@ -266,6 +292,7 @@
       const int tgt = f + D;
       if constexpr (!NOW) {
         if (tgt < N1) ring[(N2 + tgt) % F] = ldw1(wp, tgt);
+        else if (SCHED != 0 && next_sel && tgt - N1 < DX) ring[(N2 + tgt) % F] = __builtin_bit_cast(u32x4, __builtin_amdgcn_raw_buffer_load_b128(nrs0, lane16, nexts + (unsigned)(tgt - N1) * 1024u, 0));
         else if (has_next && tgt - N1 < DX) ring[(N2 + tgt) % F] = ldw2(nexts, tgt - N1);
       }
       __builtin_amdgcn_sched_barrier(0);
@@ -336,6 +363,90 @@
     if (k <= NCH) __syncthreads();
   };
   static_assert(NCH >= 4, "steady intervals");
+  u32x2 xr[4][NI2];
+  auto ld_xr = [&]() __attribute__((always_inline)) {
+    const int l_ = lane_now(), rb = 64 * mh + (l_ & 15), nc = (C / 4) * nq + 4 * NI2 * (l_ >> 4);
+#pragma unroll
+    for (int i = 0; i < 4; ++i) { const int m = m0 + rb + 16 * i, ms = m < p.M ? (p.xres_rows > 0 ? m % p.xres_rows : m) : 0; load_row_chunk<NI2>(p.xres + (long long)ms * C + nc, xr[i]); }
+  };
+  if constexpr (SCHED != 0) {
+  auto w1s_of = [&](int k) __attribute__((always_inline)) { return (unsigned)__builtin_amdgcn_readfirstlane((unsigned)(((k * 4 + nq) * KS1) * 4) * 1024u); };
+  auto w2s_of = [&](int c) __attribute__((always_inline)) { return (unsigned)__builtin_amdgcn_readfirstlane((unsigned)(((c * 4 + nq) * KS2) * NI2) * 1024u); };
+  const unsigned pws = __builtin_amdgcn_readfirstlane((unsigned)(nq * KS1 * NI2) * 1024u);
+  float cv0;
+  { const unsigned lane16 = (unsigned)lane_now() * 16u, wp0 = w1s_of(0);
+#pragma unroll
+    for (int f = 0; f < D; ++f) ring[(N2 + f) % F] = ldw1(wp0, f);
+    cv0 = cload(0); }
+  __builtin_amdgcn_sched_barrier(0);
+  panel_load_dma<C>(p.h, m0, p.M, panel, wid, lane);
+  asm volatile("s_waitcnt vmcnt(0)" ::: "memory");
+  cstore(0, cv0);
+  __syncthreads();
+  TB_TS(20);
+  panel_row_stats<C>(panel, lnst, tid, p.ln_eps);
+  TB_TS(21);
+  TB_TS(2);
+  { const float cv = cload(1);
+    gemm1(0, true, false, mh ? w1s_of(1) : w2s_of(0), 0, true);
+    __syncthreads();
+    TB_TS(22);
+    if (mh == 0) geglu(0);
+    cstore(1, cv);
+    __syncthreads(); }
+  if (mh == 0) {
+    for (int k = 1; k < NCH; ++k) {
+      const unsigned w1s = w1s_of(k), w2ns = w2s_of(k);
+      const bool cn = k + 1 < NCH;
+      float cv = 0.f;
+      if (k == 2) TB_TS(3);
+      if (cn) cv = cload(k + 1);
+      gemm2(k - 1, true, 1, w1s);
+      TB_TS(10);
+      gemm1(k, true, true, w2ns);
+      TB_TS(11);
+      geglu(k);
+      TB_TS(12);
+      if (cn) cstore(k + 1, cv);
+      __syncthreads();
+      TB_TS(13);
+    }
+    TB_TS(4);
+    gemm2(NCH - 1, true, 3, pws);
+    ld_xr();
+    __syncthreads();
+    TB_TS(5);
+  } else {
+    { const float cv = cload(2);
+      geglu(0);
+      gemm1(1, false, true, w2s_of(0), DX);
+      cstore(2, cv);
+      __syncthreads(); }
+    TB_TS(3);
+    for (int k = 2; k < NCH; ++k) {
+      const bool cn = k + 1 < NCH;
+      float cv = 0.f;
+      if (cn) cv = cload(k + 1);
+      geglu(k - 1);
+      TB_TS(12);
+      const unsigned w1s = w1s_of(k), w2ns = w2s_of(k - 1);
+      gemm2(k - 2, true, 1, w1s);
+      TB_TS(10);
+      gemm1(k, true, true, w2ns);
+      TB_TS(11);
+      if (cn) cstore(k + 1, cv);
+      __syncthreads();
+      TB_TS(13);
+    }
+    TB_TS(4);
+    geglu(NCH - 1);
+    gemm2(NCH - 2, true, 2, w2s_of(NCH - 1));
+    ld_xr();
+    __syncthreads();
+    gemm2(NCH - 1, true, 3, pws, true);
+    TB_TS(5);
+  }
+  } else {
   TB_TS(2);
 #pragma unroll 1
   for (int k = 0; k < 2; ++k) interval(k);
@@ -380,6 +491,7 @@
 #pragma unroll 1
   for (int k = NCH; k <= NCH + 1; ++k) interval(k);
   TB_TS(5);
+  }
 
   const int l_e = lane_now(), q = l_e >> 4, px = l_e & 15;
   const int rbase = 64 * mh + px;
@@ -390,7 +502,8 @@
   constexpr bool premul = POST == 2;
   static_assert(F == TB_F, "the proj_out stage reuses the weight ring");
   const unsigned pwbase = __builtin_amdgcn_readfirstlane((unsigned)(nq * KS1 * NI2) * 1024u);
-  if (post) panel_gemm_head<C>(ring, p.wpf, pwbase, lane16);
+  if constexpr (SCHED == 0) { if (post) panel_gemm_head<C>(ring, p.wpf, pwbase, lane16); }
+  TB_TS(50);
   if constexpr (!premul) {
   float b2v[NI2 * 4];
 #pragma unroll
@@ -414,16 +527,21 @@
   }
   if constexpr (post) {
   if constexpr (!premul) __syncthreads();
-  u32x2 xr[4][NI2];
-  auto ld_xr = [&]() __attribute__((always_inline)) {
-#pragma unroll
-    for (int i = 0; i < 4; ++i) { const int m = m0 + rbase + 16 * i, ms = m < p.M ? (p.xres_rows > 0 ? m % p.xres_rows : m) : 0; load_row_chunk<NI2>(p.xres + (long long)ms * C + ncol0, xr[i]); }
-  };
+  float bpv[NI2 * 4];
+  if constexpr (SCHED == 0) {
   ld_xr();
+  TB_TS(51);
   panel_gemm_body<C, !premul>(ring, acc2, p.wpf, pwbase, lane16, xrow, XOff<C>(q, px));
-  float bpv[NI2 * 4];
 #pragma unroll
   for (int t = 0; t < NI2; ++t) *(f32x4*)&bpv[4 * t] = *(const f32x4*)(p.bp + ncol0 + 4 * t);
+  } else {
+  TB_TS(51);
+  panel_gemm_body<C, false>(ring, acc2, p.wpf, pwbase, lane16, xrow, XOff<C>(q, px), (unsigned)(C * C * 2), [&]() __attribute__((always_inline)) {
+#pragma unroll
+    for (int t = 0; t < NI2; ++t) *(f32x4*)&bpv[4 * t] = *(const f32x4*)(p.bp + ncol0 + 4 * t);
+  });
+  }
+  TB_TS(52);
   float cs[NI2 * 4], cq[NI2 * 4];
 #pragma unroll
   for (int e = 0; e < NI2 * 4; ++e) { cs[e] = 0.f; cq[e] = 0.f; }
@@ -447,18 +565,23 @@
     }
     if (live) store_row_chunk<NI2>(p.pout + mo, pkk);
   }
+  TB_TS(53);
   if (p.colstat) {
 #pragma unroll
     for (int e = 0; e < NI2 * 4; ++e) {
+      if constexpr (SCHED == 0) {
 #pragma unroll
       for (int o = 1; o < 16; o <<= 1) { cs[e] += __shfl_xor(cs[e], o); cq[e] += __shfl_xor(cq[e], o); }
-    }
+      } else { cs[e] = row16_sum_dpp(cs[e]); cq[e] = row16_sum_dpp(cq[e]); }
+    }
+    TB_TS(54);
     float* stg = (float*)hbuf;
     if (px == 0) {
 #pragma unroll
       for (int e = 0; e < NI2 * 4; ++e) { stg[(mh * C + ncol0 + e) * 2] = cs[e]; stg[(mh * C + ncol0 + e) * 2 + 1] = cq[e]; }
     }
     __syncthreads();
+    TB_TS(55);
     if (tid < C) {
       float* op = p.colstat + ((long long)blockIdx.x * C + tid) * 2;
       op[0] = stg[tid * 2] + stg[(C + tid) * 2]; op[1] = stg[tid * 2 + 1] + stg[(C + tid) * 2 + 1];
@@ -476,6 +599,7 @@
   const void* kfn = p.wpf ? (p.premul ? (const void*)ff_fused_kernel<320, 0, 2> : (const void*)ff_fused_kernel<320, 0, 1>) : (const void*)ff_fused_kernel<320>;
   if (p.wpf && (!p.bp || !p.xres || !p.pout)) { agd_set_error("ff_fused: the proj_out stage needs bias, residual and output"); return -1; }
   if (p.premul && !p.wpf) { agd_set_error("ff_fused: the pre-multiplied form is the proj_out stage's"); return -1; }
+  if (p.wpf && p.premul && p.sched2) kfn = (const void*)ff_fused_kernel<320, 0, 2, 1>;
 #ifdef AGD_EXPERIMENTS
   static const void* const vars[16] = {(const void*)ff_fused_kernel<320, 0>, (const void*)ff_fused_kernel<320, 1>, (const void*)ff_fused_kernel<320, 2>, (const void*)ff_fused_kernel<320, 3>,
                                        (const void*)ff_fused_kernel<320, 4>, nullptr, (const void*)ff_fused_kernel<320, 6>, (const void*)ff_fused_kernel<320, 7>,
diff --git a/agenda_amd/ops.py b/agenda_amd/ops.py
--- a/agenda_amd/ops.py
+++ b/agenda_amd/ops.py
@@ -75,6 +75,21 @@
                                    _lib.ptr(_f32c(w2)), _lib.ptr(_f32c(b2)), _lib.ptr(y), x2.shape[0], Cc, float(eps),
                                    _lib.current_stream_ptr()), None, "agd_op_ff_fused")
     return y.reshape(x.shape)
+
+
+def ff_fused_proj(x, gamma, beta, w1, b1, w2, b2, wp, bp, xres, eps=1e-5, colstat=False, sched2=True):
+    lib = _lib.load()
+    Cc = x.shape[-1]
+    x2, xr = _f32c(x).reshape(-1, Cc), _f32c(xres).reshape(-1, Cc)
+    wp, w2, b2, bp = _f32c(wp), _f32c(w2), _f32c(b2), _f32c(bp)
+    w2p, bpp = (wp.double() @ w2.double()).float().contiguous(), (wp.double() @ b2.double() + bp.double()).float().contiguous()
+    M = x2.shape[0]
+    y = torch.empty_like(x2)
+    cst = torch.zeros((M + 127) // 128, Cc, 2, device=x2.device, dtype=torch.float32) if colstat else None
+    _lib.check(lib.agd_op_ff_fused_proj(_lib.ptr(x2), _lib.ptr(_f32c(gamma)), _lib.ptr(_f32c(beta)), _lib.ptr(_f32c(w1)), _lib.ptr(_f32c(b1)), _lib.ptr(w2p), _lib.ptr(bpp),
+                                        _lib.ptr(wp), _lib.ptr(xr), _lib.ptr(y), _lib.ptr(cst), M, Cc, xr.shape[0], float(eps), int(bool(sched2)), _lib.current_stream_ptr()),
+               None, "agd_op_ff_fused_proj")
+    return (y, cst) if colstat else y
 
 
 def attn_chain(x, gamma, beta, wq, kv, wo, bo, heads=8, eps=1e-5, return_probs=False, rows32=False):
diff --git a/include/agenda_hip.h b/include/agenda_hip.h
--- a/include/agenda_hip.h
+++ b/include/agenda_hip.h
@@ -194,6 +194,8 @@
                   int N, int geglu, void* stream);
 int agd_op_ff_fused(const float* x, const float* gamma, const float* beta, const float* w1, const float* b1, const float* w2,
                     const float* b2, float* y, int M, int C, float eps, void* stream);
+int agd_op_ff_fused_proj(const float* x, const float* gamma, const float* beta, const float* w1, const float* b1, const float* w2p, const float* bpp, const float* wp,
+                         const float* xres, float* y, float* colstat, int M, int C, int xres_rows, float eps, int sched2, void* stream);
 int agd_op_attn_chain(const float* x, const float* gamma, const float* beta, const float* wq, const float* kv, const float* wo,
                       const float* bo, float* y, float* probs_sum, int B, int HW, int T, int C, int heads, float eps, void* stream);
 int agd_op_xattn_premul(const float* x, const float* gamma, const float* beta, const float* wq, const float* kv, const float* wo,
```
